# qirui-chen/RGA3-release

Measured on AMD Instinct MI355X. Metric: video-QA samples/sec (fwd+bwd) at 7B/16-frame — full RGA3 training step (Qwen2.5-VL-7B + SAM2-L + mask losses + AdamW), higher is better.
Workload: dtype bf16

## Files before the change

### include/rga3_hip.h

```cpp
#ifndef RGA3_HIP_H
#define RGA3_HIP_H

#include <stddef.h>
#include <stdint.h>

#ifdef __cplusplus
extern "C" {
#endif

#define RGA3_EINVAL (-22)

#define RGA3_BF16 0
#define RGA3_F32 1

#define RGA3_ACT_NONE 0
#define RGA3_ACT_GELU 1
#define RGA3_ACT_SWIGLU 2
#define RGA3_ACT_RELU 3

int rga3_version(void);
int rga3_last_error(char* buf, size_t n);

int rga3_gemm_bf16(const void* A, const void* W, const void* bias, const void* residual, const void* colscale, void* C, int64_t M, int64_t N,
                   int64_t K, int64_t lda, int64_t ldw, int64_t ldc, int64_t ldr, int act, int out_dtype, int tile,
                   void* workspace, int64_t workspace_bytes, void* stream);
int rga3_gemm_rms_bf16(const void* A, const void* W, const void* bias, const void* residual, void* C, int64_t M, int64_t N, int64_t K, int64_t lda,
                       int64_t ldw, int64_t ldc, int64_t ldr, int act, int tile, void* workspace, int64_t workspace_bytes, const uint64_t* row_sumsq_in,
                       int64_t norm_width, float eps, uint64_t* row_sumsq_out, void* stream);
int rga3_gemm_swiglu_pre_bf16(const void* A, const void* W, const void* bias, void* C, void* pre, int64_t M, int64_t N, int64_t K, int64_t lda, int64_t ldw,
                              int64_t ldc, int64_t ldpre, int tile, void* workspace, int64_t workspace_bytes, void* stream);
int rga3_gemm_cat_bf16(const void* A, const void* W, const void* bias, void* C, int64_t M, int64_t N, int64_t K, int64_t lda, int64_t ldw, int64_t ldc,
                       const void* A2, const void* W2, int64_t K2, int64_t lda2, int64_t ldw2, const void* Wn, void* Cn, int64_t N2, int64_t ldwn, int64_t ldcn,
                       int tile, void* stream);

int64_t rga3_gemm_workspace_bytes(void);
int rga3_gemm_tn_bf16(const void* A, const void* B, const void* bias, void* C, int64_t M, int64_t N, int64_t K, int64_t lda, int64_t ldb,
                      int64_t ldc, int out_dtype, void* workspace, int64_t workspace_bytes, void* counters, void* stream);
int rga3_gemm_tn_many(const void* const* ptrs, const int64_t* dims, int n, void* workspace, int64_t workspace_bytes, void* stream);


int rga3_attn_varlen_fwd(const void* q, const void* k, const void* v, void* o, float* lse, const int32_t* cu_q,
                         const int32_t* cu_k, int nseg, int max_q, int64_t total_q, int Hq, int Hkv, int D, int64_t q_st, int64_t q_sh,
                         int64_t k_st, int64_t k_sh, int64_t v_st, int64_t v_sh, int64_t o_st, int64_t o_sh,
                         float scale, int causal, int impl, float* split_ws, int64_t split_ws_elems, int max_k, int block_q, int block_k, void* stream);
int rga3_attn_varlen_fwd_rope(const void* q, const void* k, const void* v, void* o, float* lse, const int32_t* cu_q, const int32_t* cu_k, int nseg, int max_q,
                              int64_t total_q, int Hq, int Hkv, int D, int64_t q_st, int64_t q_sh, int64_t k_st, int64_t k_sh, int64_t v_st, int64_t v_sh,
                              int64_t o_st, int64_t o_sh, float scale, int causal, const float* cos_q, const float* sin_q, const float* cos_k,
                              const float* sin_k, void* stream);

int rga3_rmsnorm_fwd(const void* x, const void* add, const void* weight, void* y, void* res_out, int64_t rows,
                     int64_t dim, int64_t ldx, float eps, void* stream);

int rga3_layernorm_fwd(const void* x, const void* weight, const void* bias, void* y, int64_t rows, int64_t dim,
                       int64_t ldx, int64_t ldy, float eps, int act, void* stream);
int rga3_layernorm_stats(const void* x, float* stats, int64_t rows, int64_t dim, int64_t ldx, float eps, void* stream);
int rga3_gemm_ln_bf16(const void* A, const void* Wf, const void* bias, const float* colc, const float* rowstat, void* C, int64_t M, int64_t N, int64_t K,
                      int64_t lda, int64_t ldw, int64_t ldc, int act, int tile, void* stream);
int64_t rga3_gemm_lnsum_slices(int64_t N, int tile);
int rga3_gemm_lnsum_bf16(const void* A, const void* W, const void* bias, const void* residual, void* C, int64_t M, int64_t N, int64_t K, int64_t lda,
                         int64_t ldw, int64_t ldc, int64_t ldr, int tile, float* row_parts, void* stream);
int rga3_gemm_lnq_bf16(const void* A, const void* Wf, const void* bias, const float* colc, const float* row_parts, int64_t slices, int64_t norm_width, float eps,
                       void* C, int64_t M, int64_t N, int64_t K, int64_t lda, int64_t ldw, int64_t ldc, int act, int tile, void* stream);

int rga3_rope_inplace(void* x, const float* cos, const float* sin, int64_t T, int h0, int nh, int D, int64_t st,
                      int64_t sh, void* stream);

int rga3_gather_rows(const void* table, const int64_t* idx, void* out, int64_t n_idx, int64_t rows_per_idx,
                     int64_t dim, int64_t ld_table, int64_t ld_out, void* stream);
int rga3_scatter_rows(const void* src, const int64_t* idx, void* out, int64_t n_idx, int64_t rows_per_idx, int64_t dim,
                      int64_t ld_src, int64_t ld_out, void* stream);

int rga3_pad_cols(const void* src, void* dst, int64_t rows, int64_t cols, int64_t ld_src, int64_t ld_dst, void* stream);

int rga3_silu_mul(const void* a, const void* b, void* out, int64_t n, void* stream);
int rga3_add(const void* a, const void* b, void* out, int64_t n, void* stream);

int rga3_cross_entropy_rows(const void* logits, int logits_dtype, const int64_t* labels, float* row_loss,
                            void* dlogits, int64_t rows, int64_t V, int64_t ld, float grad_scale, void* stream);


int rga3_im2col(const void* img, void* out, int64_t F, int C, int H, int W, int ks, int stride, int pad, int64_t ld_out,
                void* stream);
int rga3_maxpool2x2_win(const void* x, void* y, int64_t nwin, int w, int C, int64_t ldx, int64_t ldy, void* stream);
int rga3_upsample2x_add(const void* a, const void* b, void* out, int64_t F, int H, int W, int C, void* stream);
int rga3_add_bcast(const void* a, const void* b, void* out, int64_t rows, int64_t rows_b, int C, int64_t lda, int64_t ldb,
                   int64_t ldo, float alpha, void* stream);
int rga3_bilinear(const void* in, int in_dtype, float* out, const int32_t* plane_idx, int64_t N, int Hi, int Wi, int Ho, int Wo,
                  void* stream);
int rga3_conv3x3s2(const void* x, int x_dtype, const void* w, const void* bias, void* y, int64_t F, int H, int W, int Cin, int Cout,
                   float sig_scale, float sig_bias, void* stream);
int rga3_decimg_rows(const void* keys, int64_t keys_stride, const void* pe, int64_t pe_stride, int hw, const void* kt, const void* vt, int nk, const void* wq, const void* bq,
                     const void* wo, const void* bo, const void* ln_w, const void* ln_b, float eps, const void* wk2, const void* bk2, const void* wv2, const void* bv2,
                     void* keys_out, int64_t keys_out_stride, void* k2, void* v2, int64_t kv_stride, int v2_transposed, float scale, int64_t M, void* stream);
int rga3_attn_fewq(const void* q, int64_t q_stride, const void* k, int64_t k_stride, int64_t k_head_stride, const void* vt, const void* vbias, void* out, int64_t out_stride,
                   int frames, int nq, int nk, int H, float scale, void* stream);
int rga3_copy_many(void* const* dst, const void* const* src, const int64_t* bytes, int n, void* stream);
int rga3_conv3x3s2_ln_gelu(const void* x, int x_dtype, const void* w, const void* bias, const void* ln_w, const void* ln_b, float eps, void* y, int64_t F, int H, int W,
                           int Cin, int Cout, float sig_scale, float sig_bias, void* stream);
int rga3_im2col3x3s2(const void* x, void* cols, int64_t F, int H, int W, int C, void* stream);
int rga3_dwconv7x7(const void* x, const void* w, const void* bias, void* y, int64_t F, int H, int W, int C, void* stream);
int rga3_rope_axial_inplace(void* x, const float* cos, const float* sin, int64_t n_rope, int nq, int C, int64_t ldx, void* stream);
int rga3_pixel_shuffle2x(const void* g, const void* bias, const void* add, void* out, int64_t F, int H, int W, int Co, int act, void* stream);
int rga3_bce_dice_sums(const float* logits, const float* targets, float* out4, int64_t n_masks, int64_t hw, void* stream);
int64_t rga3_bce_dice_sums_ws_floats(int64_t n_masks, int64_t hw);
int rga3_bce_dice_sums_det(const float* logits, const float* targets, float* out4, float* ws, int64_t ws_floats, int64_t n_masks, int64_t hw, void* stream);
int64_t rga3_mask_jf_ws_bytes(int64_t frames, int64_t h, int64_t w);
int rga3_mask_jf_counts(const void* seg, const void* ann, const void* void_pixels, int64_t* counts, void* ws, int64_t ws_bytes, int64_t frames, int64_t h, int64_t w,
                        int radius, void* stream);
int64_t rga3_stom_ws_bytes(int64_t frames, int64_t h, int64_t w);
int rga3_stom_flow(const float* tracks, const void* visibility, int* records, int64_t frames, int64_t n_points, int vip_frame_idx, void* stream);
int rga3_stom_shift_composite(const void* frames_u8, const void* overlay_rgba, const int* records, void* out, int64_t frames, int64_t h, int64_t w, int vip_frame_idx,
                              void* stream);
int rga3_stom_mask_composite(const void* frames_u8, const void* overlay_rgba, const float* tracks, const void* visibility, void* out, void* ws, int64_t ws_bytes,
                             int64_t frames, int64_t h, int64_t w, int64_t n_points, int vip_frame_idx, const void* spans, int ksize, const void* half_widths,
                             int radius, void* stream);


int rga3_attn_varlen_bwd(const void* q, const void* k, const void* v, const void* o, const void* dout, const float* lse, void* dq,
                         void* dk, void* dv, float* delta_ws, const int32_t* cu_q, const int32_t* cu_k, int nseg, int max_q,
                         int max_k, int64_t total_q, int Hq, int Hkv, int D, const int64_t* strides16, float scale, int causal,
                         float* dkv_ws, int64_t total_k, void* stream);
int rga3_hiera_mlp144(const void* x, const void* w1f, const float* c1, const void* d1, const void* w2, const void* b2, void* y, int64_t M, float eps, void* stream);
int64_t rga3_hiera_mlp288_pack_bytes(void);
int rga3_hiera_mlp288_pack(const void* w1f, const float* c1, const void* d1, const void* w2, void* pack, void* stream);
int rga3_hiera_mlp288(const void* x, const void* pack, const void* b2, void* y, int64_t M, float eps, void* stream);
int rga3_mlp3_rows(const void* const* ptrs, const int64_t* dims, int n, int64_t B, void* stream);
int rga3_sam_select_objptr(const void* iou, const void* obj, const void* toks, int64_t tok_bstride, int C, const void* w0, const void* b0, const void* w1, const void* b1,
                           const void* w2, const void* b2, const void* no_obj_ptr, int64_t* best, int32_t* sel, void* obj_ptr, int64_t B, void* stream);
int64_t rga3_memattn_cross_ws_floats(int64_t Nq, int nsplit);
int rga3_memattn_cross(const void* q, const void* k, const void* m, void* out, int64_t Nq, int64_t Nk, int64_t q_stride, int64_t k_stride, int64_t m_stride,
                       int64_t out_stride, float scale, int nsplit, float* ws, void* stream);
int rga3_memlayer_rows(const void* a, int64_t a_stride, int K1, const float* part_o, const float* part_ml, int nsplit, const void* w1, const void* b1,
                       const void* res, int64_t res_stride, void* x_out, int64_t x_stride, const void* ln_w, const void* ln_b, float eps, void* t_out,
                       int64_t t_stride, const void* w2, const void* b2, int N2, void* y_out, int64_t y_stride, const float* cos, const float* sin,
                       int rope_cols, int nq, int64_t M, void* stream);
int rga3_gemm_rows16_many(const void* const* ptrs, const int64_t* dims, int n, void* stream);
int rga3_gemm_stream_k_timeouts(const void* workspace);
int64_t rga3_gemm_timeout_counter_offset(void);
int rga3_gemm_ragged_plan(int64_t M, int64_t N, int64_t K, int cus, int split, int* plan, unsigned* start);
int rga3_gemm_tiles(int entry, int* ids, int* bm, int* bn, int cap);
int rga3_gemm_candidates(int entry, int64_t M, int64_t N, int64_t K, int act, int out_dtype, int epilogue, int* ids, int cap);
int rga3_gemm_tn_slices(int64_t M, int64_t N, int64_t K);
int rga3_rmsnorm_bwd(const void* x, const void* weight, const void* dy, const void* add, void* dx, int64_t rows, int64_t dim, float eps,
                     void* stream);
int rga3_dropout_bf16(const void* x, void* y, int64_t n, float p, int64_t seed, int accumulate, void* stream);
int rga3_dropout_pair_bf16(const void* xa, const void* xb, void* ya, void* yb, int64_t n, float pa, int64_t seed_a, float pb, int64_t seed_b, int sum, void* stream);
int rga3_swiglu_fwd(const void* gu, void* a, int64_t T, int64_t I, void* stream);
int rga3_swiglu_bwd(const void* gu, const void* da, void* dgu, int64_t T, int64_t I, void* stream);
int rga3_transpose16(const void* in, void* out, int64_t R, int64_t C, int64_t ld_in, int64_t ld_out, void* stream);
int rga3_transpose16_many(const void* const* ptrs, const int64_t* dims, int n, void* stream);
int rga3_segment_sum_rows(const void* x, const int64_t* rows, const int64_t* offsets, void* out, int64_t n_out, int64_t dim, int64_t ldx,
                          void* stream);
int rga3_adamw_step(void* param, float* master, const void* grad, float* m, float* v, int64_t n, float lr, float beta1, float beta2,
                    float eps, float weight_decay, int step, float grad_scale, void* stream);
int rga3_sumsq_accum(const void* g, float* out, int64_t n, void* stream);
int rga3_sumsq_det(const void* g, int64_t n, float* partials, int64_t partials_cap, float* out, int accumulate, void* stream);
int rga3_adamw_step_clip(void* param, float* master, const void* grad, float* m, float* v, int64_t n, float lr, float beta1, float beta2,
                         float eps, float weight_decay, int step, const float* sumsq, float max_norm, void* stream);
int rga3_adamw_step_clip_rows(void* param, float* master, const void* grad, float* m, float* v, int64_t rows, int64_t row_len, const uint8_t* row_active,
                              float lr, float beta1, float beta2, float eps, int step, const float* sumsq, float max_norm, void* stream);
int rga3_scatter_add_rows(void* dst, const int64_t* idx, const void* src, int64_t n, int64_t dim, int64_t ld_dst, int64_t ld_src, float scale,
                          void* stream);


int64_t rga3_layernorm_bwd_ws_floats(int64_t rows, int64_t dim);
int rga3_layernorm_bwd(const void* x, const void* weight, const void* dy, void* dx, float* dweight, float* dbias, int64_t rows, int64_t dim,
                       float eps, float* ws, int64_t ws_floats, void* stream);
int rga3_colsum_accum(const void* x, float* out, int64_t rows, int64_t cols, int64_t ld, void* stream);
int64_t rga3_colsum_ws_floats(int64_t rows, int64_t cols);
int rga3_colsum(const void* x, float* out, int64_t rows, int64_t cols, int64_t ld, float* ws, int64_t ws_floats, void* counters, void* stream);
int rga3_act(const void* a, const void* dy, void* out, int64_t n, int kind, void* stream);
int rga3_bilinear_bwd(const float* dout, float* din, const int32_t* plane_idx, int64_t N, int Hi, int Wi, int Ho, int Wo, void* stream);
int rga3_mask_product(const void* hyper, const void* up, float* masks, int64_t B, int64_t NM, int64_t P, int64_t C, void* stream);
int64_t rga3_mask_product_bwd_ws_floats(int64_t B, int64_t NM, int64_t P, int64_t C);
int rga3_mask_product_bwd(const float* dmasks, const void* hyper, const void* up, void* dup, void* dhyper, int64_t B, int64_t NM, int64_t P, int64_t C,
                          float* ws, int64_t ws_floats, void* stream);
int rga3_pixel_shuffle2x_bwd(const void* dout, void* dg, int64_t F, int H, int W, int Co, void* stream);
int rga3_bce_dice_grad(const float* logits, const float* targets, const float* sums4, float* dlogits, int64_t n_masks, int64_t hw,
                       float coef_bce, float coef_dice, void* stream);
int rga3_bce_dice_grad_dev(const float* logits, const float* targets, const float* sums4, float* dlogits, int64_t n_masks, int64_t hw,
                           const float* coef_bce_dev, const float* coef_dice_dev, void* stream);

int rga3_pil_bicubic_coeffs(int in_size, int out_size, int32_t* bounds, int32_t* kk, int64_t kk_capacity, int* ksize_out);
int rga3_sam_preprocess_u8(const void* frames, int64_t T, int H, int W, int out_h, int out_w, const int32_t* bh, const int32_t* kh,
                           int ksize_h, const int32_t* bv, const int32_t* kv, int ksize_v, void* tmp, void* dst_u8, void* dst_bf16,
                           const float* mean3, const float* std3, void* stream);

int rga3_qwen_norm_lut(const float* mean3, const float* std3, int fused, float* lut768);
int rga3_qwen_patchify_u8(const void* frames, int64_t T, int h, int w, const float* lut768, void* out, int out_dtype, int patch, int tpatch,
                          int merge, void* stream);

int rga3_quant_fp8_rows(const void* x, void* q, float* scales, int64_t rows, int64_t K, int64_t ldx, int64_t ldq, void* stream);
int rga3_gemm_fp8(const void* Aq, const void* Wq, const float* sa, const float* sw, const void* bias, const void* residual, void* C, int64_t M,
                  int64_t N, int64_t K, int64_t lda, int64_t ldw, int64_t ldc, int64_t ldr, void* stream);
int rga3_swiglu_fwd_quant_fp8(const void* gu, void* q, float* scales, int64_t T, int64_t I, void* stream);
int rga3_swiglu_bwd_quant_fp8(const void* gu, const void* da, void* q, float* scales, int64_t T, int64_t I, void* stream);

#ifdef __cplusplus
}
#endif
#endif
```

### rga3-release_amd/csrc/attn_bwd.hip

```cpp
#include "common.h"

namespace rga3 {

struct AttnBwdArgs {
    const unsigned short *q, *k, *v, *o, *dout;
    unsigned short *dq, *dk, *dv;
    const float* lse;
    float* delta;
    const int *cu_q, *cu_k;
    long q_st, q_sh, k_st, k_sh, v_st, v_sh, o_st, o_sh, do_st, do_sh, dq_st, dq_sh, dk_st, dk_sh, dv_st, dv_sh;
    int Hq, Hkv, D;
    long total_q;
    float scale, scale_log2;
    int causal;
    float* dkv_ws;
    long total_k;
    int gx, gy;
};

constexpr int BT = 64;

template <int DP, int QT, int NWAVE, bool PAIR>
__global__ __launch_bounds__(64 * NWAVE) void attn_bwd_dq_kernel(AttnBwdArgs p) {
    constexpr int NT = 64 * NWAVE;
    constexpr int BLOCK_M = NWAVE * QT * 16;
    constexpr int CH = DP / 8;
    constexpr int STRIDE = DP * 2 + 32;
    constexpr int DS = DP / 32, DT = DP / 16;
    constexpr int LOADS = (BT * CH) / NT;
    static_assert((BT * CH) % NT == 0, "tile chunks must divide evenly over threads");

    extern __shared__ __attribute__((aligned(16))) char smem[];
    char* Ks = smem;
    char* Vs = smem + BT * STRIDE;

    const int tid = threadIdx.x, lane = tid & 63;
    const int wid = __builtin_amdgcn_readfirstlane(tid >> 6);
    const int g = lane >> 4, c = lane & 15;
    const Wg3 wg = xcd_decode3(p.gx, p.gy);
    const int seg = wg.z, hq = wg.y;
    const int hk = hq / (p.Hq / p.Hkv);
    const int qs = p.cu_q[seg], Lq = p.cu_q[seg + 1] - qs;
    const int ks = p.cu_k[seg], Lk = p.cu_k[seg + 1] - ks;
    const int shift = Lk - Lq;
    const int nqb = (Lq + BLOCK_M - 1) / BLOCK_M;
    int qb_first = wg.x, qb_second = -1;
    if constexpr (PAIR) {
        qb_first = nqb - 1 - wg.x;
        qb_second = wg.x;
        if (qb_second > qb_first) return;
        if (qb_second == qb_first) qb_second = -1;
    } else if (qb_first >= nqb) {
        return;
    }
    for (int pass = 0; pass < (PAIR ? 2 : 1); ++pass) {
    const int qbi = pass == 0 ? qb_first : qb_second;
    if (qbi < 0) break;
    if (pass == 1) __syncthreads();
    const int qb0 = qbi * BLOCK_M;
    const int qw0 = qb0 + wid * (QT * 16);

    bf16x8 qf[QT][DS], dof[QT][DS];
    float lse2[QT], dl[QT];
#pragma unroll
    for (int t = 0; t < QT; ++t) {
        const int qi = qw0 + t * 16 + c;
        const bool ok = qi < Lq;
#pragma unroll
        for (int ds = 0; ds < DS; ++ds) {
            const int d = ds * 32 + g * 8;
            u32x4 z = {0u, 0u, 0u, 0u}, y = {0u, 0u, 0u, 0u};
            if (ok && d < p.D) {
                z = *(const u32x4*)(p.q + (long)(qs + qi) * p.q_st + (long)hq * p.q_sh + d);
                y = *(const u32x4*)(p.dout + (long)(qs + qi) * p.do_st + (long)hq * p.do_sh + d);
            }
            qf[t][ds] = __builtin_bit_cast(bf16x8, z);
            dof[t][ds] = __builtin_bit_cast(bf16x8, y);
        }
        lse2[t] = ok ? p.lse[(long)hq * p.total_q + qs + qi] * 1.4426950408889634f : 0.f;
    }
#pragma unroll
    for (int t = 0; t < QT; ++t) {
        const int qi = qw0 + t * 16 + c;
        const bool ok = qi < Lq;
        float dp = 0.f;
#pragma unroll
        for (int ds = 0; ds < DS; ++ds) {
            const int d = ds * 32 + g * 8;
            if (ok && d < p.D) {
                const u32x4 ov = *(const u32x4*)(p.o + (long)(qs + qi) * p.o_st + (long)hq * p.o_sh + d);
                const u32x4 dv = __builtin_bit_cast(u32x4, dof[t][ds]);
#pragma unroll
                for (int i = 0; i < 4; ++i) {
                    dp += __uint_as_float(ov[i] << 16) * __uint_as_float(dv[i] << 16);
                    dp += __uint_as_float(ov[i] & 0xffff0000u) * __uint_as_float(dv[i] & 0xffff0000u);
                }
            }
        }
        dp += __shfl_xor(dp, 16, 64);
        dp += __shfl_xor(dp, 32, 64);
        dl[t] = ok ? dp : 0.f;
        if (ok && g == 0) p.delta[(long)hq * p.total_q + qs + qi] = dp;
    }

    f32x4 dqacc[QT][DT];
#pragma unroll
    for (int t = 0; t < QT; ++t)
#pragma unroll
        for (int d = 0; d < DT; ++d) dqacc[t][d] = f32x4{0.f, 0.f, 0.f, 0.f};

    int kv_end = Lk;
    if (p.causal) kv_end = min(Lk, qb0 + BLOCK_M + shift);
    if (kv_end < 0) kv_end = 0;
    const int ntiles = (kv_end + BT - 1) / BT;

    u32x4 kreg[LOADS], vreg[LOADS];
    auto load_tile = [&](int kt) {
#pragma unroll
        for (int i = 0; i < LOADS; ++i) {
            const int idx = tid + i * NT;
            const int r = idx / CH, ch = idx % CH;
            const int key = kt * BT + r;
            u32x4 zk = {0u, 0u, 0u, 0u}, zv = {0u, 0u, 0u, 0u};
            if (key < Lk && ch * 8 < p.D) {
                zk = *(const u32x4*)(p.k + (long)(ks + key) * p.k_st + (long)hk * p.k_sh + ch * 8);
                zv = *(const u32x4*)(p.v + (long)(ks + key) * p.v_st + (long)hk * p.v_sh + ch * 8);
            }
            kreg[i] = zk;
            vreg[i] = zv;
        }
    };
    auto store_tile = [&]() {
#pragma unroll
        for (int i = 0; i < LOADS; ++i) {
            const int idx = tid + i * NT;
            const int r = idx / CH, ch = idx % CH;
            *(u32x4*)(Ks + r * STRIDE + ch * 16) = kreg[i];
            *(u32x4*)(Vs + r * STRIDE + ch * 16) = vreg[i];
        }
    };

    if (ntiles > 0) load_tile(0);
    for (int kt = 0; kt < ntiles; ++kt) {
        __syncthreads();
        store_tile();
        __syncthreads();
        if (kt + 1 < ntiles) load_tile(kt + 1);
        const int k0 = kt * BT;
        const bool need_mask = (k0 + BT > Lk) || (p.causal && (k0 + BT - 1 > qb0 + shift));
#pragma unroll
        for (int t = 0; t < QT; ++t) {
            const int qi = qw0 + t * 16 + c;
            f32x4 s[4], dp[4];
#pragma unroll
            for (int j = 0; j < 4; ++j) { s[j] = f32x4{0.f, 0.f, 0.f, 0.f}; dp[j] = f32x4{0.f, 0.f, 0.f, 0.f}; }
#pragma unroll
            for (int j = 0; j < 4; ++j)
#pragma unroll
                for (int ds = 0; ds < DS; ++ds) {
                    bf16x8 kf = *(const bf16x8*)(Ks + (j * 16 + c) * STRIDE + ds * 64 + g * 16);
                    bf16x8 vf = *(const bf16x8*)(Vs + (j * 16 + c) * STRIDE + ds * 64 + g * 16);
                    s[j] = __builtin_amdgcn_mfma_f32_16x16x32_bf16(kf, qf[t][ds], s[j], 0, 0, 0);
                    dp[j] = __builtin_amdgcn_mfma_f32_16x16x32_bf16(vf, dof[t][ds], dp[j], 0, 0, 0);
                }
            bf16x8 dsf[2];
#pragma unroll
            for (int ss = 0; ss < 2; ++ss) {
                float e[8];
#pragma unroll
                for (int u = 0; u < 8; ++u) {
                    const int j = 2 * ss + (u >> 2), r = u & 3;
                    float pr = __builtin_amdgcn_exp2f(s[j][r] * p.scale_log2 - lse2[t]);
                    if (need_mask) {
                        const int key = k0 + j * 16 + 4 * g + r;
                        const bool ok = (key < Lk) && (!p.causal || key <= qi + shift);
                        pr = ok ? pr : 0.f;
                    }
                    if (qi >= Lq) pr = 0.f;
                    e[u] = pr * (dp[j][r] - dl[t]) * p.scale;
                }
                u32x4 pk;
                pk[0] = pack_bf2(e[0], e[1]); pk[1] = pack_bf2(e[2], e[3]); pk[2] = pack_bf2(e[4], e[5]); pk[3] = pack_bf2(e[6], e[7]);
                dsf[ss] = __builtin_bit_cast(bf16x8, pk);
            }
#pragma unroll
            for (int d = 0; d < DT; ++d)
#pragma unroll
                for (int ss = 0; ss < 2; ++ss) {
                    const char* a0 = Ks + (ss * 32 + 4 * g + (c >> 2)) * STRIDE + (d * 16 + 4 * (c & 3)) * 2;
                    bf16x4 lo = __builtin_amdgcn_ds_read_tr16_b64_v4bf16((__attribute__((address_space(3))) bf16x4*)(a0));
                    bf16x4 hi = __builtin_amdgcn_ds_read_tr16_b64_v4bf16((__attribute__((address_space(3))) bf16x4*)(a0 + 16 * STRIDE));
                    bf16x8 kt8;
                    kt8[0] = lo[0]; kt8[1] = lo[1]; kt8[2] = lo[2]; kt8[3] = lo[3];
                    kt8[4] = hi[0]; kt8[5] = hi[1]; kt8[6] = hi[2]; kt8[7] = hi[3];
                    dqacc[t][d] = __builtin_amdgcn_mfma_f32_16x16x32_bf16(kt8, dsf[ss], dqacc[t][d], 0, 0, 0);
                }
        }
    }
#pragma unroll
    for (int t = 0; t < QT; ++t) {
        const int qi = qw0 + t * 16 + c;
        if (qi < Lq) {
            unsigned short* row = p.dq + (long)(qs + qi) * p.dq_st + (long)hq * p.dq_sh;
#pragma unroll
            for (int d = 0; d < DT; ++d) {
                const int dd = d * 16 + 4 * g;
                if (dd < p.D) {
                    u32x2 pk;
                    pk[0] = pack_bf2(dqacc[t][d][0], dqacc[t][d][1]);
                    pk[1] = pack_bf2(dqacc[t][d][2], dqacc[t][d][3]);
                    *(u32x2*)(row + dd) = pk;
                }
            }
        }
    }
    }
}

template <int DP, int NWAVE, bool SPLIT, bool PAIR>
__global__ __launch_bounds__(64 * NWAVE) void attn_bwd_dkv_kernel(AttnBwdArgs p) {
    constexpr int NT = 64 * NWAVE;
    constexpr int BLOCK_N = NWAVE * 16;
    constexpr int CH = DP / 8;
    constexpr int STRIDE = DP * 2 + 32;
    constexpr int DS = DP / 32, DT = DP / 16;
    constexpr int LOADS = (BT * CH) / NT;
    static_assert((BT * CH) % NT == 0, "tile chunks must divide evenly over threads");

    extern __shared__ __attribute__((aligned(16))) char smem[];
    char* Qs = smem;
    char* Os = smem + BT * STRIDE;
    float* Ls = (float*)(smem + 2 * BT * STRIDE);

    const int tid = threadIdx.x, lane = tid & 63;
    const int wid = __builtin_amdgcn_readfirstlane(tid >> 6);
    const int g = lane >> 4, c = lane & 15;
    const Wg3 wg = xcd_decode3(p.gx, p.gy);
    const int seg = wg.z;
    const int group = p.Hq / p.Hkv;
    const int hk = SPLIT ? wg.y / group : wg.y;
    const int hh0 = SPLIT ? wg.y % group : 0, hh1 = SPLIT ? hh0 + 1 : group;
    const int qs = p.cu_q[seg], Lq = p.cu_q[seg + 1] - qs;
    const int ks = p.cu_k[seg], Lk = p.cu_k[seg + 1] - ks;
    const int shift = Lk - Lq;
    const int nkb = (Lk + BLOCK_N - 1) / BLOCK_N;
    int kb_first = wg.x, kb_second = -1;
    if constexpr (PAIR) {
        kb_first = wg.x;
        kb_second = nkb - 1 - wg.x;
        if (kb_first > kb_second) return;
        if (kb_second == kb_first) kb_second = -1;
    } else if (kb_first >= nkb) {
        return;
    }
    for (int pass = 0; pass < (PAIR ? 2 : 1); ++pass) {
    const int kbi = pass == 0 ? kb_first : kb_second;
    if (kbi < 0) break;
    if (pass == 1) __syncthreads();
    const int kb0 = kbi * BLOCK_N;
    const int key = kb0 + wid * 16 + c;

    bf16x8 kf[DS], vf[DS];
#pragma unroll
    for (int ds = 0; ds < DS; ++ds) {
        const int d = ds * 32 + g * 8;
        u32x4 z = {0u, 0u, 0u, 0u}, y = {0u, 0u, 0u, 0u};
        if (key < Lk && d < p.D) {
            z = *(const u32x4*)(p.k + (long)(ks + key) * p.k_st + (long)hk * p.k_sh + d);
            y = *(const u32x4*)(p.v + (long)(ks + key) * p.v_st + (long)hk * p.v_sh + d);
        }
        kf[ds] = __builtin_bit_cast(bf16x8, z);
        vf[ds] = __builtin_bit_cast(bf16x8, y);
    }
    f32x4 dkacc[DT], dvacc[DT];
#pragma unroll
    for (int d = 0; d < DT; ++d) { dkacc[d] = f32x4{0.f, 0.f, 0.f, 0.f}; dvacc[d] = f32x4{0.f, 0.f, 0.f, 0.f}; }

    int q_begin = 0;
    if (p.causal) q_begin = max(0, kb0 - shift);
    const int t0 = q_begin / BT;
    const int ntq = (Lq + BT - 1) / BT;

    u32x4 qreg[LOADS], oreg[LOADS];
    float lreg = 0.f, dreg = 0.f;
    auto load_tile = [&](int hq_, int qt_) {
#pragma unroll
        for (int i = 0; i < LOADS; ++i) {
            const int idx = tid + i * NT;
            const int r = idx / CH, ch = idx % CH;
            const int qi = qt_ * BT + r;
            u32x4 zq = {0u, 0u, 0u, 0u}, zo = {0u, 0u, 0u, 0u};
            if (qi < Lq && ch * 8 < p.D) {
                zq = *(const u32x4*)(p.q + (long)(qs + qi) * p.q_st + (long)hq_ * p.q_sh + ch * 8);
                zo = *(const u32x4*)(p.dout + (long)(qs + qi) * p.do_st + (long)hq_ * p.do_sh + ch * 8);
            }
            qreg[i] = zq;
            oreg[i] = zo;
        }
        if (tid < BT) {
            const int qi = qt_ * BT + tid;
            lreg = (qi < Lq) ? p.lse[(long)hq_ * p.total_q + qs + qi] * 1.4426950408889634f : 0.f;
            dreg = (qi < Lq) ? p.delta[(long)hq_ * p.total_q + qs + qi] : 0.f;
        }
    };
    auto store_tile = [&]() {
#pragma unroll
        for (int i = 0; i < LOADS; ++i) {
            const int idx = tid + i * NT;
            const int r = idx / CH, ch = idx % CH;
            *(u32x4*)(Qs + r * STRIDE + ch * 16) = qreg[i];
            *(u32x4*)(Os + r * STRIDE + ch * 16) = oreg[i];
        }
        if (tid < BT) {
            Ls[tid] = lreg;
            Ls[BT + tid] = dreg;
        }
    };
    if (t0 < ntq) load_tile(hk * group + hh0, t0);
    for (int hh = hh0; hh < hh1; ++hh) {
        const int hq = hk * group + hh;
        for (int qt = t0; qt < ntq; ++qt) {
            __syncthreads();
            store_tile();
            __syncthreads();
            if (qt + 1 < ntq) load_tile(hq, qt + 1);
            else if (hh + 1 < hh1) load_tile(hq + 1, t0);
            const int q0 = qt * BT;
            f32x4 s[4], dp[4];
#pragma unroll
            for (int j = 0; j < 4; ++j) { s[j] = f32x4{0.f, 0.f, 0.f, 0.f}; dp[j] = f32x4{0.f, 0.f, 0.f, 0.f}; }
#pragma unroll
            for (int j = 0; j < 4; ++j)
#pragma unroll
                for (int ds = 0; ds < DS; ++ds) {
                    bf16x8 qa = *(const bf16x8*)(Qs + (j * 16 + c) * STRIDE + ds * 64 + g * 16);
                    bf16x8 oa = *(const bf16x8*)(Os + (j * 16 + c) * STRIDE + ds * 64 + g * 16);
                    s[j] = __builtin_amdgcn_mfma_f32_16x16x32_bf16(qa, kf[ds], s[j], 0, 0, 0);
                    dp[j] = __builtin_amdgcn_mfma_f32_16x16x32_bf16(oa, vf[ds], dp[j], 0, 0, 0);
                }
            bf16x8 pf[2], dsf[2];
#pragma unroll
            for (int ss = 0; ss < 2; ++ss) {
                float e[8], f[8];
#pragma unroll
                for (int u = 0; u < 8; ++u) {
                    const int j = 2 * ss + (u >> 2), r = u & 3;
                    const int ql = j * 16 + 4 * g + r;
                    const int qi = q0 + ql;
                    float pr = __builtin_amdgcn_exp2f(s[j][r] * p.scale_log2 - Ls[ql]);
                    const bool ok = (qi < Lq) && (key < Lk) && (!p.causal || key <= qi + shift);
                    pr = ok ? pr : 0.f;
                    e[u] = pr;
                    f[u] = pr * (dp[j][r] - Ls[BT + ql]) * p.scale;
                }
                u32x4 a, b;
                a[0] = pack_bf2(e[0], e[1]); a[1] = pack_bf2(e[2], e[3]); a[2] = pack_bf2(e[4], e[5]); a[3] = pack_bf2(e[6], e[7]);
                b[0] = pack_bf2(f[0], f[1]); b[1] = pack_bf2(f[2], f[3]); b[2] = pack_bf2(f[4], f[5]); b[3] = pack_bf2(f[6], f[7]);
                pf[ss] = __builtin_bit_cast(bf16x8, a);
                dsf[ss] = __builtin_bit_cast(bf16x8, b);
            }
#pragma unroll
            for (int d = 0; d < DT; ++d)
#pragma unroll
                for (int ss = 0; ss < 2; ++ss) {
                    const int roff = (ss * 32 + 4 * g + (c >> 2)) * STRIDE + (d * 16 + 4 * (c & 3)) * 2;
                    bf16x4 ol = __builtin_amdgcn_ds_read_tr16_b64_v4bf16((__attribute__((address_space(3))) bf16x4*)(Os + roff));
                    bf16x4 oh = __builtin_amdgcn_ds_read_tr16_b64_v4bf16((__attribute__((address_space(3))) bf16x4*)(Os + roff + 16 * STRIDE));
                    bf16x4 ql_ = __builtin_amdgcn_ds_read_tr16_b64_v4bf16((__attribute__((address_space(3))) bf16x4*)(Qs + roff));
                    bf16x4 qh_ = __builtin_amdgcn_ds_read_tr16_b64_v4bf16((__attribute__((address_space(3))) bf16x4*)(Qs + roff + 16 * STRIDE));
                    bf16x8 ot, qt8;
                    ot[0] = ol[0]; ot[1] = ol[1]; ot[2] = ol[2]; ot[3] = ol[3]; ot[4] = oh[0]; ot[5] = oh[1]; ot[6] = oh[2]; ot[7] = oh[3];
                    qt8[0] = ql_[0]; qt8[1] = ql_[1]; qt8[2] = ql_[2]; qt8[3] = ql_[3]; qt8[4] = qh_[0]; qt8[5] = qh_[1]; qt8[6] = qh_[2]; qt8[7] = qh_[3];
                    dvacc[d] = __builtin_amdgcn_mfma_f32_16x16x32_bf16(ot, pf[ss], dvacc[d], 0, 0, 0);
                    dkacc[d] = __builtin_amdgcn_mfma_f32_16x16x32_bf16(qt8, dsf[ss], dkacc[d], 0, 0, 0);
                }
        }
    }
    if constexpr (SPLIT) {
        if (key < Lk) {
            const long half = (long)group * p.total_k * p.Hkv * p.D;
            float* wk = p.dkv_ws + (((long)hh0 * p.total_k + ks + key) * p.Hkv + hk) * p.D;
#pragma unroll
            for (int d = 0; d < DT; ++d) {
                const int dd = d * 16 + 4 * g;
                if (dd < p.D) {
                    *(f32x4*)(wk + dd) = dkacc[d];
                    *(f32x4*)(wk + half + dd) = dvacc[d];
                }
            }
        }
        continue;
    }
    if (key < Lk) {
        unsigned short* rk = p.dk + (long)(ks + key) * p.dk_st + (long)hk * p.dk_sh;
        unsigned short* rv = p.dv + (long)(ks + key) * p.dv_st + (long)hk * p.dv_sh;
#pragma unroll
        for (int d = 0; d < DT; ++d) {
            const int dd = d * 16 + 4 * g;
            if (dd < p.D) {
                u32x2 a, b;
                a[0] = pack_bf2(dkacc[d][0], dkacc[d][1]); a[1] = pack_bf2(dkacc[d][2], dkacc[d][3]);
                b[0] = pack_bf2(dvacc[d][0], dvacc[d][1]); b[1] = pack_bf2(dvacc[d][2], dvacc[d][3]);
                *(u32x2*)(rk + dd) = a;
                *(u32x2*)(rv + dd) = b;
            }
        }
    }
    }
}

__global__ __launch_bounds__(256) void attn_dkv_reduce_kernel(AttnBwdArgs p) {
    const int group = p.Hq / p.Hkv;
    const int d4 = p.D / 4;
    const long idx = (long)blockIdx.x * 256 + threadIdx.x;
    const long total = p.total_k * p.Hkv * d4;
    if (idx >= total) return;
    const int dd = (int)(idx % d4) * 4;
    const long row = idx / d4;
    const int hk = (int)(row % p.Hkv);
    const long key = row / p.Hkv;
    const long plane = p.total_k * p.Hkv * (long)p.D, half = (long)group * plane;
    const float* w = p.dkv_ws + row * p.D + dd;
    f32x4 sk = *(const f32x4*)w, sv = *(const f32x4*)(w + half);
    for (int h = 1; h < group; ++h) {
        sk += *(const f32x4*)(w + h * plane);
        sv += *(const f32x4*)(w + half + h * plane);
    }
    u32x2 a, b;
    a[0] = pack_bf2(sk[0], sk[1]); a[1] = pack_bf2(sk[2], sk[3]);
    b[0] = pack_bf2(sv[0], sv[1]); b[1] = pack_bf2(sv[2], sv[3]);
    *(u32x2*)(p.dk + key * p.dk_st + (long)hk * p.dk_sh + dd) = a;
    *(u32x2*)(p.dv + key * p.dv_st + (long)hk * p.dv_sh + dd) = b;
}

template <auto K>
static int launch_bwd_grid(AttnBwdArgs& a, int lds, unsigned gx, int gy, int nseg, int nwave, hipStream_t st, const char* name) {
    a.gx = (int)gx; a.gy = gy;
    return launch_lds<K>(dim3(gx * (unsigned)gy * (unsigned)nseg), dim3(64 * nwave), lds, st, name, a);
}

template <int DP>
static int launch_bwd(const AttnBwdArgs& a0, int nseg, int max_q, int max_k, hipStream_t st) {
    AttnBwdArgs a = a0;
    a.gx = 1; a.gy = 1;
    constexpr int NW = (DP == 128) ? 8 : 4;
#ifdef RGA3_BWD_DQ_QT2
    constexpr int QT = 2, NWQ = 4;
#else
    constexpr int QT = (DP >= 128) ? 1 : 2, NWQ = NW;
#endif
    constexpr int BLOCK_M = NWQ * QT * 16;
    constexpr int LDS_DQ = 2 * BT * (DP * 2 + 32);
    constexpr int LDS_DKV = 2 * BT * (DP * 2 + 32) + 2 * BT * 4;
    const unsigned nqb = (unsigned)cdiv(max_q, BLOCK_M), nkb = (unsigned)cdiv(max_k, 16 * NW);
    const bool pair = a.causal && nqb >= 4 && nkb >= 4;
    const unsigned gq = pair ? (nqb + 1) / 2 : nqb, gk = pair ? (nkb + 1) / 2 : nkb;
    if (int rc = pair ? launch_bwd_grid<attn_bwd_dq_kernel<DP, QT, NWQ, true>>(a, LDS_DQ, gq, a.Hq, nseg, NWQ, st, "attn_bwd_dq_kernel")
                      : launch_bwd_grid<attn_bwd_dq_kernel<DP, QT, NWQ, false>>(a, LDS_DQ, gq, a.Hq, nseg, NWQ, st, "attn_bwd_dq_kernel"))
        return rc;
    if (a.dkv_ws && a.Hq > a.Hkv) {
        if (int rc = pair ? launch_bwd_grid<attn_bwd_dkv_kernel<DP, NW, true, true>>(a, LDS_DKV, gk, a.Hq, nseg, NW, st, "attn_bwd_dkv_kernel<split>")
                          : launch_bwd_grid<attn_bwd_dkv_kernel<DP, NW, true, false>>(a, LDS_DKV, gk, a.Hq, nseg, NW, st, "attn_bwd_dkv_kernel<split>"))
            return rc;
        const long rows = a.total_k * a.Hkv;
        hipLaunchKernelGGL(attn_dkv_reduce_kernel, dim3((unsigned)cdiv(rows * (a.D / 4), 256)), dim3(256), 0, st, a);
        RGA3_CHECK_LAUNCH("attn_dkv_reduce_kernel");
        return 0;
    }
    return pair ? launch_bwd_grid<attn_bwd_dkv_kernel<DP, NW, false, true>>(a, LDS_DKV, gk, a.Hkv, nseg, NW, st, "attn_bwd_dkv_kernel")
                : launch_bwd_grid<attn_bwd_dkv_kernel<DP, NW, false, false>>(a, LDS_DKV, gk, a.Hkv, nseg, NW, st, "attn_bwd_dkv_kernel");
}

}

using namespace rga3;

extern "C" int rga3_attn_varlen_bwd(const void* q, const void* k, const void* v, const void* o, const void* dout, const float* lse,
                                    void* dq, void* dk, void* dv, float* delta_ws, const int32_t* cu_q, const int32_t* cu_k, int nseg,
                                    int max_q, int max_k, int64_t total_q, int Hq, int Hkv, int D, const int64_t* strides16, float scale,
                                    int causal, float* dkv_ws, int64_t total_k, void* stream) {
    RGA3_CHECK_ARG(q && k && v && o && dout && lse && dq && dk && dv && delta_ws && cu_q && cu_k && strides16, "attn_bwd: null pointer");
    RGA3_CHECK_ARG(nseg > 0 && max_q > 0 && max_k > 0 && total_q > 0, "attn_bwd: sizes");
    RGA3_CHECK_ARG(Hq > 0 && Hkv > 0 && Hq % Hkv == 0, "attn_bwd: Hq=%d Hkv=%d", Hq, Hkv);
    RGA3_CHECK_ARG(D >= 8 && D <= 128 && D % 8 == 0, "attn_bwd: head dim %d unsupported (multiple of 8, <= 128)", D);
    for (int i = 0; i < 16; ++i) RGA3_CHECK_ARG(strides16[i] % 4 == 0, "attn_bwd: stride %d must be a multiple of 4 elements", i);
    for (int i = 0; i < 10; ++i) RGA3_CHECK_ARG(strides16[i] % 8 == 0, "attn_bwd: input stride %d must be a multiple of 8 elements", i);
    {
        static const char* const names[8] = {"q", "k", "v", "o", "dout", "dq", "dk", "dv"};
        for (int i = 0; i < 8; ++i) {
            const bool kv = i == 1 || i == 2 || i == 6 || i == 7;
            RGA3_CHECK_HEADS("attn_bwd", names[i], strides16[2 * i], strides16[2 * i + 1], kv ? total_k : total_q, kv ? Hkv : Hq, D);
        }
    }
    AttnBwdArgs a;
    a.q = (const unsigned short*)q; a.k = (const unsigned short*)k; a.v = (const unsigned short*)v; a.o = (const unsigned short*)o;
    a.dout = (const unsigned short*)dout; a.dq = (unsigned short*)dq; a.dk = (unsigned short*)dk; a.dv = (unsigned short*)dv;
    a.lse = lse; a.delta = delta_ws; a.cu_q = cu_q; a.cu_k = cu_k;
    a.q_st = strides16[0]; a.q_sh = strides16[1]; a.k_st = strides16[2]; a.k_sh = strides16[3]; a.v_st = strides16[4]; a.v_sh = strides16[5];
    a.o_st = strides16[6]; a.o_sh = strides16[7]; a.do_st = strides16[8]; a.do_sh = strides16[9]; a.dq_st = strides16[10]; a.dq_sh = strides16[11];
    a.dk_st = strides16[12]; a.dk_sh = strides16[13]; a.dv_st = strides16[14]; a.dv_sh = strides16[15];
    a.Hq = Hq; a.Hkv = Hkv; a.D = D; a.total_q = total_q; a.scale = scale; a.scale_log2 = scale * 1.4426950408889634f; a.causal = causal;
    a.dkv_ws = dkv_ws; a.total_k = total_k;
    RGA3_CHECK_ARG(!dkv_ws || (total_k > 0 && D % 4 == 0), "attn_bwd: dkv_ws needs total_k");
    hipStream_t st = (hipStream_t)stream;
    if (D <= 32) return launch_bwd<32>(a, nseg, max_q, max_k, st);
    if (D <= 64) return launch_bwd<64>(a, nseg, max_q, max_k, st);
    if (D <= 96) return launch_bwd<96>(a, nseg, max_q, max_k, st);
    return launch_bwd<128>(a, nseg, max_q, max_k, st);
}
```

### rga3-release_amd/csrc/trainops.hip

```cpp
#include "common.h"

namespace rga3 {

template <int MAXC>
__global__ __launch_bounds__(256) void rmsnorm_bwd_kernel(const unsigned short* __restrict__ x, const unsigned short* __restrict__ w,
                                                          const unsigned short* __restrict__ dy, const unsigned short* __restrict__ add,
                                                          unsigned short* __restrict__ dx, long rows, int dim, float eps) {
    const int lane = threadIdx.x & 63;
    const long row = (long)blockIdx.x * 4 + (threadIdx.x >> 6);
    if (row >= rows) return;
    const int nch = dim / 8;
    u32x4 xb[MAXC], gb[MAXC];
    float ss = 0.f, sg = 0.f;
#pragma unroll
    for (int i = 0; i < MAXC; ++i) {
        const int ch = lane + i * 64;
        if (ch < nch) {
            float fx[8], fd[8], fw[8];
            xb[i] = *(const u32x4*)(x + row * dim + ch * 8);
            unpack8(xb[i], fx);
            unpack8(*(const u32x4*)(dy + row * dim + ch * 8), fd);
            unpack8(*(const u32x4*)(w + ch * 8), fw);
#pragma unroll
            for (int e = 0; e < 8; ++e) {
                fd[e] *= fw[e];
                ss += fx[e] * fx[e];
                sg += fd[e] * fx[e];
            }
            gb[i] = pack8(fd);
        }
    }
    ss = wave_sum(ss);
    sg = wave_sum(sg);
    const float r = rsqrtf(ss / (float)dim + eps);
    const float coef = r * r * r * sg / (float)dim;
#pragma unroll
    for (int i = 0; i < MAXC; ++i) {
        const int ch = lane + i * 64;
        if (ch < nch) {
            float fx[8], fg[8], fa[8];
            unpack8(xb[i], fx);
            unpack8(gb[i], fg);
            if (add) unpack8(*(const u32x4*)(add + row * dim + ch * 8), fa);
#pragma unroll
            for (int e = 0; e < 8; ++e) fg[e] = r * fg[e] - fx[e] * coef + (add ? fa[e] : 0.f);
            *(u32x4*)(dx + row * dim + ch * 8) = pack8(fg);
        }
    }
}

template <int NC>
__global__ __launch_bounds__(256) void rmsnorm_bwd_block_kernel(const unsigned short* __restrict__ x, const unsigned short* __restrict__ w,
                                                                const unsigned short* __restrict__ dy, const unsigned short* __restrict__ add,
                                                                unsigned short* __restrict__ dx, int dim, float eps) {
    __shared__ float red[2][4];
    const int lane = threadIdx.x & 63, wv = threadIdx.x >> 6;
    const long row = blockIdx.x;
    const int nch = dim / 8;
    float fx[NC][8], fg[NC][8];
    float ss = 0.f, sg = 0.f;
#pragma unroll
    for (int i = 0; i < NC; ++i) {
        const int ch = threadIdx.x + i * 256;
        if (ch < nch) {
            float fw[8];
            unpack8(*(const u32x4*)(x + row * dim + ch * 8), fx[i]);
            unpack8(*(const u32x4*)(dy + row * dim + ch * 8), fg[i]);
            unpack8(*(const u32x4*)(w + ch * 8), fw);
#pragma unroll
            for (int e = 0; e < 8; ++e) {
                fg[i][e] *= fw[e];
                ss += fx[i][e] * fx[i][e];
                sg += fg[i][e] * fx[i][e];
            }
        }
    }
    ss = wave_sum(ss);
    sg = wave_sum(sg);
    if (lane == 0) { red[0][wv] = ss; red[1][wv] = sg; }
    __syncthreads();
    ss = (red[0][0] + red[0][1]) + (red[0][2] + red[0][3]);
    sg = (red[1][0] + red[1][1]) + (red[1][2] + red[1][3]);
    const float r = rsqrtf(ss / (float)dim + eps);
    const float coef = r * r * r * sg / (float)dim;
#pragma unroll
    for (int i = 0; i < NC; ++i) {
        const int ch = threadIdx.x + i * 256;
        if (ch < nch) {
            float fa[8], o[8];
            if (add) unpack8(*(const u32x4*)(add + row * dim + ch * 8), fa);
#pragma unroll
            for (int e = 0; e < 8; ++e) o[e] = r * fg[i][e] - fx[i][e] * coef + (add ? fa[e] : 0.f);
            *(u32x4*)(dx + row * dim + ch * 8) = pack8(o);
        }
    }
}

__global__ __launch_bounds__(256) void swiglu_bwd_kernel(const unsigned short* __restrict__ gu, const unsigned short* __restrict__ da,
                                                         unsigned short* __restrict__ dgu, long T, long I) {
    const long nch = I / 8;
    const long total = T * nch;
    for (long i = (long)blockIdx.x * 256 + threadIdx.x; i < total; i += (long)gridDim.x * 256) {
        const long ch = i % nch, t = i / nch;
        const long blk = ch / 2, half = ch % 2;
        const long goff = t * 2 * I + blk * 32 + half * 8;
        float g[8], u[8], d[8], dg[8], du[8];
        unpack8(*(const u32x4*)(gu + goff), g);
        unpack8(*(const u32x4*)(gu + goff + 16), u);
        unpack8(*(const u32x4*)(da + t * I + ch * 8), d);
#pragma unroll
        for (int e = 0; e < 8; ++e) swiglu_bwd_elem(g[e], u[e], d[e], dg[e], du[e]);
        *(u32x4*)(dgu + goff) = pack8(dg);
        *(u32x4*)(dgu + goff + 16) = pack8(du);
    }
}

__global__ __launch_bounds__(256) void swiglu_fwd_kernel(const unsigned short* __restrict__ gu, unsigned short* __restrict__ a, long T, long I) {
    const long nch = I / 8;
    const long total = T * nch;
    for (long i = (long)blockIdx.x * 256 + threadIdx.x; i < total; i += (long)gridDim.x * 256) {
        const long ch = i % nch, t = i / nch;
        const long blk = ch / 2, half = ch % 2;
        const long goff = t * 2 * I + blk * 32 + half * 8;
        float g[8], u[8], o[8];
        unpack8(*(const u32x4*)(gu + goff), g);
        unpack8(*(const u32x4*)(gu + goff + 16), u);
#pragma unroll
        for (int e = 0; e < 8; ++e) o[e] = swiglu_fwd_elem(g[e], u[e]);
        *(u32x4*)(a + t * I + ch * 8) = pack8(o);
    }
}

__global__ __launch_bounds__(256) void transpose16_kernel(const unsigned short* __restrict__ in, unsigned short* __restrict__ out, long R, long C,
                                                          long ldi, long ldo) {
    __shared__ unsigned short tile[64][66];
    const long r0 = (long)blockIdx.y * 64, c0 = (long)blockIdx.x * 64;
    const int tx = threadIdx.x & 63, ty = threadIdx.x >> 6;
    for (int i = ty; i < 64; i += 4) {
        const long r = r0 + i, c = c0 + tx;
        tile[i][tx] = (r < R && c < C) ? in[r * ldi + c] : (unsigned short)0;
    }
    __syncthreads();
    for (int i = ty; i < 64; i += 4) {
        const long c = c0 + i, r = r0 + tx;
        if (c < C && r < R) out[c * ldo + r] = tile[tx][i];
    }
}

constexpr int TR_MANY = 64;
struct TransposeMany {
    const unsigned short* in[TR_MANY];
    unsigned short* out[TR_MANY];
    int R[TR_MANY], C[TR_MANY];
};
__global__ __launch_bounds__(256) void transpose16_many_kernel(TransposeMany p) {
    __shared__ unsigned short tile[64][66];
    const int m = blockIdx.z;
    const long R = p.R[m], C = p.C[m];
    const long r0 = (long)blockIdx.y * 64, c0 = (long)blockIdx.x * 64;
    if (r0 >= R || c0 >= C) return;
    const unsigned short* in = p.in[m];
    unsigned short* out = p.out[m];
    const int tx = threadIdx.x & 63, ty = threadIdx.x >> 6;
    for (int i = ty; i < 64; i += 4) {
        const long r = r0 + i, c = c0 + tx;
        tile[i][tx] = (r < R && c < C) ? in[r * C + c] : (unsigned short)0;
    }
    __syncthreads();
    for (int i = ty; i < 64; i += 4) {
        const long c = c0 + i, r = r0 + tx;
        if (c < C && r < R) out[c * R + r] = tile[tx][i];
    }
}

__global__ __launch_bounds__(256) void segment_sum_rows_kernel(const unsigned short* __restrict__ x, const long* __restrict__ rows,
                                                               const long* __restrict__ off, unsigned short* __restrict__ out, int dim, long ldx) {
    const long u = blockIdx.x;
    const long a = off[u], b = off[u + 1];
    for (int ch = threadIdx.x; ch < dim / 8; ch += 256) {
        float acc[8] = {0, 0, 0, 0, 0, 0, 0, 0};
        for (long j = a; j < b; ++j) {
            float f[8];
            unpack8(*(const u32x4*)(x + rows[j] * ldx + ch * 8), f);
#pragma unroll
            for (int e = 0; e < 8; ++e) acc[e] += f[e];
        }
        *(u32x4*)(out + u * dim + ch * 8) = pack8(acc);
    }
}

__global__ __launch_bounds__(256) void adamw_kernel(unsigned short* __restrict__ p, float* __restrict__ master, const unsigned short* __restrict__ g,
                                                    float* __restrict__ m, float* __restrict__ v, long n, float lr, float b1, float b2, float eps,
                                                    float wd, float bc1, float bc2, float gscale) {
    for (long i = (long)blockIdx.x * 256 + threadIdx.x; i < n; i += (long)gridDim.x * 256) {
        const float gr = bf2f(g[i]) * gscale;
        float w = master[i];
        const float mi = b1 * m[i] + (1.f - b1) * gr;
        const float vi = b2 * v[i] + (1.f - b2) * gr * gr;
        m[i] = mi;
        v[i] = vi;
        w = w * (1.f - lr * wd) - lr * (mi / bc1) / (sqrtf(vi / bc2) + eps);
        master[i] = w;
        p[i] = f2bf(w);
    }
}

__global__ __launch_bounds__(256) void sumsq_kernel(const unsigned short* __restrict__ g, float* __restrict__ out, long n) {
    __shared__ float red[4];
    float s = 0.f;
    for (long i = (long)blockIdx.x * 256 + threadIdx.x; i < n; i += (long)gridDim.x * 256) {
        const float x = bf2f(g[i]);
        s += x * x;
    }
    s = wave_sum(s);
    if ((threadIdx.x & 63) == 0) red[threadIdx.x >> 6] = s;
    __syncthreads();
    if (threadIdx.x == 0) atomicAdd(out, red[0] + red[1] + red[2] + red[3]);
}

__global__ __launch_bounds__(256) void sumsq_partials_kernel(const unsigned short* __restrict__ g, float* __restrict__ partials, long n) {
    __shared__ float red[4];
    float s = 0.f;
    const long n8 = n / 8;
    for (long i = (long)blockIdx.x * 256 + threadIdx.x; i < n8; i += (long)gridDim.x * 256) {
        float f[8];
        unpack8(*(const u32x4*)(g + i * 8), f);
#pragma unroll
        for (int e = 0; e < 8; ++e) s += f[e] * f[e];
    }
    if (blockIdx.x == 0 && threadIdx.x < (n & 7)) {
        const float x = bf2f(g[n8 * 8 + threadIdx.x]);
        s += x * x;
    }
    s = wave_sum(s);
    if ((threadIdx.x & 63) == 0) red[threadIdx.x >> 6] = s;
    __syncthreads();
    if (threadIdx.x == 0) partials[blockIdx.x] = (red[0] + red[1]) + (red[2] + red[3]);
}

__global__ __launch_bounds__(256) void sumsq_finish_kernel(const float* __restrict__ partials, int np, float* __restrict__ out, int accumulate) {
    __shared__ float red[256];
    float s = 0.f;
    for (int i = threadIdx.x; i < np; i += 256) s += partials[i];
    red[threadIdx.x] = s;
    __syncthreads();
    for (int o = 128; o > 0; o >>= 1) {
        if ((int)threadIdx.x < o) red[threadIdx.x] += red[threadIdx.x + o];
        __syncthreads();
    }
    if (threadIdx.x == 0) out[0] = (accumulate ? out[0] : 0.f) + red[0];
}

__global__ __launch_bounds__(256) void adamw8_kernel(unsigned short* __restrict__ p, float* __restrict__ master, const unsigned short* __restrict__ g,
                                                     float* __restrict__ m, float* __restrict__ v, long n, float lr, float b1, float b2, float eps,
                                                     float wd, float bc1, float bc2, const float* __restrict__ sumsq, float max_norm,
                                                     const unsigned char* __restrict__ row_active, long row_len8) {
    float gscale = 1.f;
    if (sumsq) gscale = fminf(1.f, max_norm / (sqrtf(sumsq[0]) + 1e-6f));
    const long n8 = n / 8;
    const float decay = 1.f - lr * wd, ibc1 = 1.f / bc1, ibc2 = 1.f / bc2;
    for (long i = (long)blockIdx.x * 256 + threadIdx.x; i < n8; i += (long)gridDim.x * 256) {
        if (row_active && !row_active[i / row_len8]) continue;
        float gr[8], w[8], mi[8], vi[8];
        unpack8(*(const u32x4*)(g + i * 8), gr);
        *(f32x4*)(w) = *(const f32x4*)(master + i * 8);     *(f32x4*)(w + 4) = *(const f32x4*)(master + i * 8 + 4);
        *(f32x4*)(mi) = *(const f32x4*)(m + i * 8);         *(f32x4*)(mi + 4) = *(const f32x4*)(m + i * 8 + 4);
        *(f32x4*)(vi) = *(const f32x4*)(v + i * 8);         *(f32x4*)(vi + 4) = *(const f32x4*)(v + i * 8 + 4);
#pragma unroll
        for (int e = 0; e < 8; ++e) {
            const float x = gr[e] * gscale;
            mi[e] = b1 * mi[e] + (1.f - b1) * x;
            vi[e] = b2 * vi[e] + (1.f - b2) * x * x;
            w[e] = w[e] * decay - lr * (mi[e] * ibc1) / (sqrtf(vi[e] * ibc2) + eps);
        }
        *(f32x4*)(master + i * 8) = *(f32x4*)(w);           *(f32x4*)(master + i * 8 + 4) = *(f32x4*)(w + 4);
        *(f32x4*)(m + i * 8) = *(f32x4*)(mi);               *(f32x4*)(m + i * 8 + 4) = *(f32x4*)(mi + 4);
        *(f32x4*)(v + i * 8) = *(f32x4*)(vi);               *(f32x4*)(v + i * 8 + 4) = *(f32x4*)(vi + 4);
        *(u32x4*)(p + i * 8) = pack8(w);
    }
    if (blockIdx.x == 0 && threadIdx.x < (n & 7)) {
        const long i = n8 * 8 + threadIdx.x;
        const float x = bf2f(g[i]) * gscale;
        const float mm = b1 * m[i] + (1.f - b1) * x, vv = b2 * v[i] + (1.f - b2) * x * x;
        const float w = master[i] * decay - lr * (mm * ibc1) / (sqrtf(vv * ibc2) + eps);
        m[i] = mm; v[i] = vv; master[i] = w; p[i] = f2bf(w);
    }
}

__global__ __launch_bounds__(256) void scatter_add_rows_kernel(unsigned short* __restrict__ dst, const long* __restrict__ idx, const unsigned short* __restrict__ src,
                                                               long n, int dim, long ld_dst, long ld_src, float scale) {
    const int nch = dim / 8;
    for (long t = (long)blockIdx.x * 256 + threadIdx.x; t < n * nch; t += (long)gridDim.x * 256) {
        const long r = t / nch;
        const int ch = (int)(t % nch);
        float a[8], b[8];
        unsigned short* d = dst + idx[r] * ld_dst + ch * 8;
        unpack8(*(const u32x4*)d, a);
        unpack8(*(const u32x4*)(src + r * ld_src + ch * 8), b);
#pragma unroll
        for (int e = 0; e < 8; ++e) a[e] += scale * b[e];
        *(u32x4*)d = pack8(a);
    }
}

__device__ __forceinline__ unsigned dropout_hash(unsigned long long seed, unsigned long long ctr) {
    unsigned x = (unsigned)ctr ^ (unsigned)seed, y = (unsigned)(ctr >> 32) ^ (unsigned)(seed >> 32);
    x *= 0xcc9e2d51u; x = (x << 15) | (x >> 17); x *= 0x1b873593u;
    y ^= x; y = (y << 13) | (y >> 19); y = y * 5u + 0xe6546b64u;
    y ^= y >> 16; y *= 0x85ebca6bu; y ^= y >> 13; y *= 0xc2b2ae35u; y ^= y >> 16;
    return y;
}

__global__ __launch_bounds__(256) void dropout_kernel(const unsigned short* __restrict__ x, unsigned short* __restrict__ y, long n8, unsigned thr,
                                                      float inv_keep, unsigned long long seed, int accumulate) {
    for (long g = (long)blockIdx.x * 256 + threadIdx.x; g < n8; g += (long)gridDim.x * 256) {
        const u32x4 v = *(const u32x4*)(x + g * 8);
        u32x4 o = {0u, 0u, 0u, 0u};
        if (accumulate) o = *(const u32x4*)(y + g * 8);
#pragma unroll
        for (int j = 0; j < 4; ++j) {
            const unsigned h = dropout_hash(seed, (unsigned long long)g * 4 + j);
            const float lo = ((h & 0xffffu) >= thr) ? __uint_as_float(v[j] << 16) * inv_keep : 0.f;
            const float hi = ((h >> 16) >= thr) ? __uint_as_float(v[j] & 0xffff0000u) * inv_keep : 0.f;
            const float alo = accumulate ? __uint_as_float(o[j] << 16) : 0.f, ahi = accumulate ? __uint_as_float(o[j] & 0xffff0000u) : 0.f;
            o[j] = pack_bf2(alo + lo, ahi + hi);
        }
        *(u32x4*)(y + g * 8) = o;
    }
}

__global__ __launch_bounds__(256) void dropout_pair_kernel(const unsigned short* __restrict__ xa, const unsigned short* __restrict__ xb, unsigned short* ya,
                                                           unsigned short* yb, long n8, unsigned thr_a, float ik_a, unsigned long long seed_a, unsigned thr_b,
                                                           float ik_b, unsigned long long seed_b, int sum) {
    const bool same = xa == xb;
    for (long g = (long)blockIdx.x * 256 + threadIdx.x; g < n8; g += (long)gridDim.x * 256) {
        const u32x4 va = *(const u32x4*)(xa + g * 8);
        const u32x4 vb = same ? va : *(const u32x4*)(xb + g * 8);
        u32x4 o = {0u, 0u, 0u, 0u};
        if (sum) o = *(const u32x4*)(ya + g * 8);
        u32x4 oa, ob;
#pragma unroll
        for (int j = 0; j < 4; ++j) {
            const unsigned ha = dropout_hash(seed_a, (unsigned long long)g * 4 + j), hb = dropout_hash(seed_b, (unsigned long long)g * 4 + j);
            const float alo = ((ha & 0xffffu) >= thr_a) ? __uint_as_float(va[j] << 16) * ik_a : 0.f;
            const float ahi = ((ha >> 16) >= thr_a) ? __uint_as_float(va[j] & 0xffff0000u) * ik_a : 0.f;
            const float blo = ((hb & 0xffffu) >= thr_b) ? __uint_as_float(vb[j] << 16) * ik_b : 0.f;
            const float bhi = ((hb >> 16) >= thr_b) ? __uint_as_float(vb[j] & 0xffff0000u) * ik_b : 0.f;
            if (sum) {
                oa[j] = pack_bf2(__uint_as_float(o[j] << 16) + alo + blo, __uint_as_float(o[j] & 0xffff0000u) + ahi + bhi);
            } else {
                oa[j] = pack_bf2(alo, ahi);
                ob[j] = pack_bf2(blo, bhi);
            }
        }
        *(u32x4*)(ya + g * 8) = oa;
        if (!sum) *(u32x4*)(yb + g * 8) = ob;
    }
}

}

using namespace rga3;

extern "C" int rga3_rmsnorm_bwd(const void* x, const void* weight, const void* dy, const void* add, void* dx, int64_t rows, int64_t dim,
                                float eps, void* stream) {
    RGA3_CHECK_ARG(x && weight && dy && dx && rows > 0 && dim > 0 && dim % 8 == 0 && dim <= 8192, "rmsnorm_bwd: bad args");
    hipStream_t st = (hipStream_t)stream;
    if (dim > 1024) {
        dim3 gb((unsigned)rows);
        if (dim <= 2048) hipLaunchKernelGGL(rmsnorm_bwd_block_kernel<1>, gb, dim3(256), 0, st, (cus)x, (cus)weight, (cus)dy, (cus)add, (us)dx, (int)dim, eps);
        else if (dim <= 4096) hipLaunchKernelGGL(rmsnorm_bwd_block_kernel<2>, gb, dim3(256), 0, st, (cus)x, (cus)weight, (cus)dy, (cus)add, (us)dx, (int)dim, eps);
        else hipLaunchKernelGGL(rmsnorm_bwd_block_kernel<4>, gb, dim3(256), 0, st, (cus)x, (cus)weight, (cus)dy, (cus)add, (us)dx, (int)dim, eps);
        RGA3_CHECK_LAUNCH("rmsnorm_bwd_block");
        return 0;
    }
    dim3 grid((unsigned)cdiv(rows, 4));
    if (dim <= 2048) hipLaunchKernelGGL(rmsnorm_bwd_kernel<4>, grid, dim3(256), 0, st, (cus)x, (cus)weight, (cus)dy, (cus)add, (us)dx, (long)rows, (int)dim, eps);
    else if (dim <= 4096) hipLaunchKernelGGL(rmsnorm_bwd_kernel<8>, grid, dim3(256), 0, st, (cus)x, (cus)weight, (cus)dy, (cus)add, (us)dx, (long)rows, (int)dim, eps);
    else hipLaunchKernelGGL(rmsnorm_bwd_kernel<16>, grid, dim3(256), 0, st, (cus)x, (cus)weight, (cus)dy, (cus)add, (us)dx, (long)rows, (int)dim, eps);
    RGA3_CHECK_LAUNCH("rmsnorm_bwd");
    return 0;
}

extern "C" int rga3_dropout_bf16(const void* x, void* y, int64_t n, float p, int64_t seed, int accumulate, void* stream) {
    RGA3_CHECK_ARG(x && y && n > 0 && n % 8 == 0, "dropout: n=%ld must be a positive multiple of 8", (long)n);
    RGA3_CHECK_ARG(p >= 0.f && p < 1.f, "dropout: p=%f", p);
    const unsigned thr = (unsigned)(p * 65536.0f + 0.5f);
    const float inv_keep = 1.0f / (1.0f - (float)thr / 65536.0f);
    long blocks = cdiv(n / 8, 256);
    if (blocks > 65536) blocks = 65536;
    hipLaunchKernelGGL(dropout_kernel, dim3((unsigned)blocks), dim3(256), 0, (hipStream_t)stream, (const unsigned short*)x, (unsigned short*)y, (long)(n / 8),
                       thr, inv_keep, (unsigned long long)seed, accumulate);
    RGA3_CHECK_LAUNCH("dropout_kernel");
    return 0;
}

extern "C" int rga3_dropout_pair_bf16(const void* xa, const void* xb, void* ya, void* yb, int64_t n, float pa, int64_t seed_a, float pb, int64_t seed_b, int sum,
                                      void* stream) {
    RGA3_CHECK_ARG(xa && xb && ya && (sum || yb) && n > 0 && n % 8 == 0, "dropout_pair: null pointer / n=%ld must be a positive multiple of 8", (long)n);
    RGA3_CHECK_ARG(pa >= 0.f && pa < 1.f && pb >= 0.f && pb < 1.f, "dropout_pair: p=%f / %f", pa, pb);
    RGA3_CHECK_ARG((((uintptr_t)xa | (uintptr_t)xb | (uintptr_t)ya | (uintptr_t)yb) & 15) == 0, "dropout_pair: pointers must be 16-byte aligned");
    const unsigned ta = (unsigned)(pa * 65536.0f + 0.5f), tb = (unsigned)(pb * 65536.0f + 0.5f);
    long blocks = cdiv(n / 8, 256);
    if (blocks > 65536) blocks = 65536;
    hipLaunchKernelGGL(dropout_pair_kernel, dim3((unsigned)blocks), dim3(256), 0, (hipStream_t)stream, (cus)xa, (cus)xb, (us)ya, (us)yb, (long)(n / 8), ta,
                       1.0f / (1.0f - (float)ta / 65536.0f), (unsigned long long)seed_a, tb, 1.0f / (1.0f - (float)tb / 65536.0f), (unsigned long long)seed_b, sum);
    RGA3_CHECK_LAUNCH("dropout_pair_kernel");
    return 0;
}

extern "C" int rga3_swiglu_bwd(const void* gu, const void* da, void* dgu, int64_t T, int64_t I, void* stream) {
    RGA3_CHECK_ARG(gu && da && dgu && T > 0 && I > 0 && I % 16 == 0, "swiglu_bwd: bad args");
    hipLaunchKernelGGL(swiglu_bwd_kernel, dim3(grid1d(T * (I / 8))), dim3(256), 0, (hipStream_t)stream, (cus)gu, (cus)da, (us)dgu, (long)T, (long)I);
    RGA3_CHECK_LAUNCH("swiglu_bwd");
    return 0;
}

extern "C" int rga3_swiglu_fwd(const void* gu, void* a, int64_t T, int64_t I, void* stream) {
    RGA3_CHECK_ARG(gu && a && T > 0 && I > 0 && I % 16 == 0, "swiglu_fwd: bad args");
    hipLaunchKernelGGL(swiglu_fwd_kernel, dim3(grid1d(T * (I / 8))), dim3(256), 0, (hipStream_t)stream, (cus)gu, (us)a, (long)T, (long)I);
    RGA3_CHECK_LAUNCH("swiglu_fwd");
    return 0;
}

extern "C" int rga3_transpose16(const void* in, void* out, int64_t R, int64_t C, int64_t ld_in, int64_t ld_out, void* stream) {
    RGA3_CHECK_ARG(in && out && R > 0 && C > 0, "transpose16: bad args");
    RGA3_CHECK_LD("transpose16", "ld_in", ld_in, C, 2);
    RGA3_CHECK_LD("transpose16", "ld_out", ld_out, R, 2);
    RGA3_CHECK_ARG(cdiv(R, 64) <= 65535, "transpose16: too many rows");
    hipLaunchKernelGGL(transpose16_kernel, dim3((unsigned)cdiv(C, 64), (unsigned)cdiv(R, 64)), dim3(256), 0, (hipStream_t)stream, (cus)in, (us)out, (long)R,
                       (long)C, (long)ld_in, (long)ld_out);
    RGA3_CHECK_LAUNCH("transpose16");
    return 0;
}

extern "C" int rga3_transpose16_many(const void* const* ptrs, const int64_t* dims, int n, void* stream) {
    RGA3_CHECK_ARG(ptrs && dims && n >= 1 && n <= TR_MANY, "transpose16_many: n %d (1..64)", n);
    TransposeMany p;
    long mr = 0, mc = 0;
    for (int i = 0; i < n; ++i) {
        p.in[i] = (const unsigned short*)ptrs[2 * i];
        p.out[i] = (unsigned short*)ptrs[2 * i + 1];
        RGA3_CHECK_ARG(p.in[i] && p.out[i] && dims[2 * i] > 0 && dims[2 * i + 1] > 0 && dims[2 * i] < (1 << 30) && dims[2 * i + 1] < (1 << 30), "transpose16_many: matrix %d", i);
        p.R[i] = (int)dims[2 * i];
        p.C[i] = (int)dims[2 * i + 1];
        if (p.R[i] > mr) mr = p.R[i];
        if (p.C[i] > mc) mc = p.C[i];
    }
    RGA3_CHECK_ARG(cdiv(mr, 64) <= 65535, "transpose16_many: too many rows");
    hipLaunchKernelGGL(transpose16_many_kernel, dim3((unsigned)cdiv(mc, 64), (unsigned)cdiv(mr, 64), (unsigned)n), dim3(256), 0, (hipStream_t)stream, p);
    RGA3_CHECK_LAUNCH("transpose16_many");
    return 0;
}

extern "C" int rga3_segment_sum_rows(const void* x, const int64_t* rows, const int64_t* offsets, void* out, int64_t n_out, int64_t dim,
                                     int64_t ldx, void* stream) {
    RGA3_CHECK_ARG(x && rows && offsets && out && n_out > 0 && dim % 8 == 0 && ldx % 8 == 0, "segment_sum_rows: bad args");
    RGA3_CHECK_LD("segment_sum_rows", "ldx", ldx, dim, 2);
    hipLaunchKernelGGL(segment_sum_rows_kernel, dim3((unsigned)n_out), dim3(256), 0, (hipStream_t)stream, (cus)x, (const long*)rows, (const long*)offsets,
                       (us)out, (int)dim, (long)ldx);
    RGA3_CHECK_LAUNCH("segment_sum_rows");
    return 0;
}

extern "C" int rga3_adamw_step(void* param, float* master, const void* grad, float* m, float* v, int64_t n, float lr, float beta1, float beta2,
                               float eps, float weight_decay, int step, float grad_scale, void* stream) {
    RGA3_CHECK_ARG(param && master && grad && m && v && n > 0 && step >= 1, "adamw_step: bad args");
    const float bc1 = 1.f - powf(beta1, (float)step), bc2 = 1.f - powf(beta2, (float)step);
    hipLaunchKernelGGL(adamw_kernel, dim3(grid1d(n)), dim3(256), 0, (hipStream_t)stream, (us)param, master, (cus)grad, m, v, (long)n, lr, beta1, beta2, eps,
                       weight_decay, bc1, bc2, grad_scale);
    RGA3_CHECK_LAUNCH("adamw_step");
    return 0;
}

extern "C" int rga3_sumsq_accum(const void* g, float* out, int64_t n, void* stream) {
    RGA3_CHECK_ARG(g && out && n > 0, "sumsq_accum: bad args");
    hipLaunchKernelGGL(sumsq_kernel, dim3(grid1d(n, 256, 2048)), dim3(256), 0, (hipStream_t)stream, (cus)g, out, (long)n);
    RGA3_CHECK_LAUNCH("sumsq_accum");
    return 0;
}

extern "C" int rga3_sumsq_det(const void* g, int64_t n, float* partials, int64_t partials_cap, float* out, int accumulate, void* stream) {
    RGA3_CHECK_ARG(g && partials && out && n > 0 && partials_cap >= 1, "sumsq_det: bad args");
    RGA3_CHECK_ARG(((uintptr_t)g & 15) == 0, "sumsq_det: gradient pointer must be 16-byte aligned");
    long nb = cdiv(n, 8 * 256 * 4);
    if (nb < 1) nb = 1;
    if (nb > partials_cap) nb = partials_cap;
    if (nb > 2048) nb = 2048;
    hipLaunchKernelGGL(sumsq_partials_kernel, dim3((unsigned)nb), dim3(256), 0, (hipStream_t)stream, (cus)g, partials, (long)n);
    RGA3_CHECK_LAUNCH("sumsq_partials");
    hipLaunchKernelGGL(sumsq_finish_kernel, dim3(1), dim3(256), 0, (hipStream_t)stream, (const float*)partials, (int)nb, out, accumulate);
    RGA3_CHECK_LAUNCH("sumsq_finish");
    return 0;
}

extern "C" int rga3_adamw_step_clip(void* param, float* master, const void* grad, float* m, float* v, int64_t n, float lr, float beta1, float beta2,
                                    float eps, float weight_decay, int step, const float* sumsq, float max_norm, void* stream) {
    RGA3_CHECK_ARG(param && master && grad && m && v && n > 0 && step >= 1, "adamw_step_clip: bad args");
    RGA3_CHECK_ARG((((uintptr_t)param | (uintptr_t)grad | (uintptr_t)master | (uintptr_t)m | (uintptr_t)v) & 15) == 0, "adamw_step_clip: pointers must be 16-byte aligned");
    const float bc1 = 1.f - powf(beta1, (float)step), bc2 = 1.f - powf(beta2, (float)step);
    hipLaunchKernelGGL(adamw8_kernel, dim3(grid1d(cdiv(n, 8), 256, 256L * 16)), dim3(256), 0, (hipStream_t)stream, (us)param, master, (cus)grad, m, v, (long)n, lr, beta1, beta2,
                       eps, weight_decay, bc1, bc2, sumsq, max_norm, (const unsigned char*)nullptr, 1L);
    RGA3_CHECK_LAUNCH("adamw_step_clip");
    return 0;
}

extern "C" int rga3_adamw_step_clip_rows(void* param, float* master, const void* grad, float* m, float* v, int64_t rows, int64_t row_len, const uint8_t* row_active,
                                         float lr, float beta1, float beta2, float eps, int step, const float* sumsq, float max_norm, void* stream) {
    RGA3_CHECK_ARG(param && master && grad && m && v && row_active && rows > 0 && row_len > 0 && row_len % 8 == 0 && step >= 1, "adamw_step_clip_rows: bad args (row_len % 8)");
    RGA3_CHECK_ARG((((uintptr_t)param | (uintptr_t)grad | (uintptr_t)master | (uintptr_t)m | (uintptr_t)v) & 15) == 0, "adamw_step_clip_rows: pointers must be 16-byte aligned");
    const float bc1 = 1.f - powf(beta1, (float)step), bc2 = 1.f - powf(beta2, (float)step);
    const int64_t n = rows * row_len;
    hipLaunchKernelGGL(adamw8_kernel, dim3(grid1d(cdiv(n, 8), 256, 256L * 16)), dim3(256), 0, (hipStream_t)stream, (us)param, master, (cus)grad, m, v, (long)n, lr, beta1, beta2,
                       eps, 0.f, bc1, bc2, sumsq, max_norm, row_active, (long)(row_len / 8));
    RGA3_CHECK_LAUNCH("adamw_step_clip_rows");
    return 0;
}

extern "C" int rga3_scatter_add_rows(void* dst, const int64_t* idx, const void* src, int64_t n, int64_t dim, int64_t ld_dst, int64_t ld_src, float scale,
                                     void* stream) {
    RGA3_CHECK_ARG(dst && idx && src && n > 0 && dim > 0 && dim % 8 == 0 && ld_dst % 8 == 0 && ld_src % 8 == 0, "scatter_add_rows: bad args");
    RGA3_CHECK_LD("scatter_add_rows", "ld_dst", ld_dst, dim, 2);
    RGA3_CHECK_LD("scatter_add_rows", "ld_src", ld_src, dim, n);
    hipLaunchKernelGGL(scatter_add_rows_kernel, dim3(grid1d(n * (dim / 8))), dim3(256), 0, (hipStream_t)stream, (us)dst, (const long*)idx, (cus)src, (long)n, (int)dim,
                       (long)ld_dst, (long)ld_src, scale);
    RGA3_CHECK_LAUNCH("scatter_add_rows");
    return 0;
}
```

### rga3-release_amd/rga3/hip/lib.py

```python
from __future__ import annotations

import ctypes as C
import os

_HERE = os.path.dirname(os.path.abspath(__file__))
LIB_PATH = os.path.normpath(os.path.join(_HERE, "..", "..", "librga3_hip.so"))

_p, _i, _i64, _f, _sz = C.c_void_p, C.c_int, C.c_int64, C.c_float, C.c_size_t

SIGNATURES = {
    "rga3_version": [],
    "rga3_last_error": [C.c_char_p, _sz],
    "rga3_gemm_bf16": [_p, _p, _p, _p, _p, _p, _i64, _i64, _i64, _i64, _i64, _i64, _i64, _i, _i, _i, _p, _i64, _p],
    "rga3_gemm_rms_bf16": [_p, _p, _p, _p, _p, _i64, _i64, _i64, _i64, _i64, _i64, _i64, _i, _i, _p, _i64, _p, _i64, _f, _p, _p],
    "rga3_gemm_workspace_bytes": [],
    "rga3_gemm_tn_bf16": [_p, _p, _p, _p, _i64, _i64, _i64, _i64, _i64, _i64, _i, _p, _i64, _p, _p],
    "rga3_gemm_tn_many": [_p, _p, _i, _p, _i64, _p],
    "rga3_gemm_swiglu_pre_bf16": [_p, _p, _p, _p, _p, _i64, _i64, _i64, _i64, _i64, _i64, _i64, _i, _p, _i64, _p],
    "rga3_gemm_cat_bf16": [_p, _p, _p, _p, _i64, _i64, _i64, _i64, _i64, _i64, _p, _p, _i64, _i64, _i64, _p, _p, _i64, _i64, _i64, _i, _p],
    "rga3_attn_varlen_fwd": [_p, _p, _p, _p, _p, _p, _p, _i, _i, _i64, _i, _i, _i, _i64, _i64, _i64, _i64, _i64, _i64,
                             _i64, _i64, _f, _i, _i, _p, _i64, _i, _i, _i, _p],
    "rga3_attn_varlen_fwd_rope": [_p, _p, _p, _p, _p, _p, _p, _i, _i, _i64, _i, _i, _i, _i64, _i64, _i64, _i64, _i64, _i64, _i64, _i64, _f, _i, _p, _p, _p, _p, _p],
    "rga3_rmsnorm_fwd": [_p, _p, _p, _p, _p, _i64, _i64, _i64, _f, _p],
    "rga3_layernorm_fwd": [_p, _p, _p, _p, _i64, _i64, _i64, _i64, _f, _i, _p],
    "rga3_layernorm_stats": [_p, _p, _i64, _i64, _i64, _f, _p],
    "rga3_gemm_ln_bf16": [_p, _p, _p, _p, _p, _p, _i64, _i64, _i64, _i64, _i64, _i64, _i, _i, _p],
    "rga3_gemm_lnsum_slices": [_i64, _i],
    "rga3_gemm_lnsum_bf16": [_p, _p, _p, _p, _p, _i64, _i64, _i64, _i64, _i64, _i64, _i64, _i, _p, _p],
    "rga3_gemm_lnq_bf16": [_p, _p, _p, _p, _p, _i64, _i64, _f, _p, _i64, _i64, _i64, _i64, _i64, _i64, _i, _i, _p],
    "rga3_rope_inplace": [_p, _p, _p, _i64, _i, _i, _i, _i64, _i64, _p],
    "rga3_gather_rows": [_p, _p, _p, _i64, _i64, _i64, _i64, _i64, _p],
    "rga3_scatter_rows": [_p, _p, _p, _i64, _i64, _i64, _i64, _i64, _p],
    "rga3_pad_cols": [_p, _p, _i64, _i64, _i64, _i64, _p],
    "rga3_silu_mul": [_p, _p, _p, _i64, _p],
    "rga3_add": [_p, _p, _p, _i64, _p],
    "rga3_cross_entropy_rows": [_p, _i, _p, _p, _p, _i64, _i64, _i64, _f, _p],
    "rga3_im2col": [_p, _p, _i64, _i, _i, _i, _i, _i, _i, _i64, _p],
    "rga3_maxpool2x2_win": [_p, _p, _i64, _i, _i, _i64, _i64, _p],
    "rga3_upsample2x_add": [_p, _p, _p, _i64, _i, _i, _i, _p],
    "rga3_add_bcast": [_p, _p, _p, _i64, _i64, _i, _i64, _i64, _i64, _f, _p],
    "rga3_bilinear": [_p, _i, _p, _p, _i64, _i, _i, _i, _i, _p],
    "rga3_conv3x3s2": [_p, _i, _p, _p, _p, _i64, _i, _i, _i, _i, _f, _f, _p],
    "rga3_decimg_rows": [_p, _i64, _p, _i64, _i, _p, _p, _i, _p, _p, _p, _p, _p, _p, _f, _p, _p, _p, _p, _p, _i64, _p, _p, _i64, _i, _f, _i64, _p],
    "rga3_attn_fewq": [_p, _i64, _p, _i64, _i64, _p, _p, _p, _i64, _i, _i, _i, _i, _f, _p],
    "rga3_copy_many": [_p, _p, _p, _i, _p],
    "rga3_conv3x3s2_ln_gelu": [_p, _i, _p, _p, _p, _p, _f, _p, _i64, _i, _i, _i, _i, _f, _f, _p],
    "rga3_dwconv7x7": [_p, _p, _p, _p, _i64, _i, _i, _i, _p],
    "rga3_rope_axial_inplace": [_p, _p, _p, _i64, _i, _i, _i64, _p],
    "rga3_pixel_shuffle2x": [_p, _p, _p, _p, _i64, _i, _i, _i, _i, _p],
    "rga3_bce_dice_sums": [_p, _p, _p, _i64, _i64, _p],
    "rga3_bce_dice_sums_ws_floats": [_i64, _i64],
    "rga3_bce_dice_sums_det": [_p, _p, _p, _p, _i64, _i64, _i64, _p],
    "rga3_mask_jf_ws_bytes": [_i64, _i64, _i64],
    "rga3_mask_jf_counts": [_p, _p, _p, _p, _p, _i64, _i64, _i64, _i64, _i, _p],
    "rga3_stom_ws_bytes": [_i64, _i64, _i64],
    "rga3_stom_flow": [_p, _p, _p, _i64, _i64, _i, _p],
    "rga3_stom_shift_composite": [_p, _p, _p, _p, _i64, _i64, _i64, _i, _p],
    "rga3_stom_mask_composite": [_p, _p, _p, _p, _p, _p, _i64, _i64, _i64, _i64, _i64, _i, _p, _i, _p, _i, _p],
    "rga3_attn_varlen_bwd": [_p, _p, _p, _p, _p, _p, _p, _p, _p, _p, _p, _p, _i, _i, _i, _i64, _i, _i, _i, _p, _f, _i, _p, _i64, _p],
    "rga3_transpose16_many": [_p, _p, _i, _p],
    "rga3_hiera_mlp144": [_p, _p, _p, _p, _p, _p, _p, _i64, _f, _p],
    "rga3_hiera_mlp288_pack_bytes": [],
    "rga3_hiera_mlp288_pack": [_p, _p, _p, _p, _p, _p],
    "rga3_hiera_mlp288": [_p, _p, _p, _p, _i64, _f, _p],
    "rga3_mlp3_rows": [_p, _p, _i, _i64, _p],
    "rga3_sam_select_objptr": [_p, _p, _p, _i64, _i, _p, _p, _p, _p, _p, _p, _p, _p, _p, _p, _i64, _p],
    "rga3_memattn_cross_ws_floats": [_i64, _i],
    "rga3_memattn_cross": [_p, _p, _p, _p, _i64, _i64, _i64, _i64, _i64, _i64, _f, _i, _p, _p],
    "rga3_memlayer_rows": [_p, _i64, _i, _p, _p, _i, _p, _p, _p, _i64, _p, _i64, _p, _p, _f, _p, _i64, _p, _p, _i, _p, _i64, _p, _p, _i, _i, _i64, _p],
    "rga3_gemm_rows16_many": [_p, _p, _i, _p],
    "rga3_gemm_stream_k_timeouts": [_p],
    "rga3_gemm_timeout_counter_offset": [],
    "rga3_gemm_ragged_plan": [_i64, _i64, _i64, _i, _i, _p, _p],
    "rga3_gemm_tiles": [_i, _p, _p, _p, _i],
    "rga3_gemm_candidates": [_i, _i64, _i64, _i64, _i, _i, _i, _p, _i],
    "rga3_gemm_tn_slices": [_i64, _i64, _i64],
    "rga3_quant_fp8_rows": [_p, _p, _p, _i64, _i64, _i64, _i64, _p],
    "rga3_gemm_fp8": [_p, _p, _p, _p, _p, _p, _p, _i64, _i64, _i64, _i64, _i64, _i64, _i64, _p],
    "rga3_swiglu_fwd_quant_fp8": [_p, _p, _p, _i64, _i64, _p],
    "rga3_swiglu_bwd_quant_fp8": [_p, _p, _p, _p, _i64, _i64, _p],
    "rga3_im2col3x3s2": [_p, _p, _i64, _i, _i, _i, _p],
    "rga3_pil_bicubic_coeffs": [_i, _i, _p, _p, _i64, _p],
    "rga3_sam_preprocess_u8": [_p, _i64, _i, _i, _i, _i, _p, _p, _i, _p, _p, _i, _p, _p, _p, _p, _p, _p],
    "rga3_qwen_norm_lut": [_p, _p, _i, _p],
    "rga3_qwen_patchify_u8": [_p, _i64, _i, _i, _p, _p, _i, _i, _i, _i, _p],
    "rga3_rmsnorm_bwd": [_p, _p, _p, _p, _p, _i64, _i64, _f, _p],
    "rga3_dropout_bf16": [_p, _p, _i64, _f, _i64, _i, _p],
    "rga3_dropout_pair_bf16": [_p, _p, _p, _p, _i64, _f, _i64, _f, _i64, _i, _p],
    "rga3_swiglu_fwd": [_p, _p, _i64, _i64, _p],
    "rga3_swiglu_bwd": [_p, _p, _p, _i64, _i64, _p],
    "rga3_transpose16": [_p, _p, _i64, _i64, _i64, _i64, _p],
    "rga3_segment_sum_rows": [_p, _p, _p, _p, _i64, _i64, _i64, _p],
    "rga3_adamw_step": [_p, _p, _p, _p, _p, _i64, _f, _f, _f, _f, _f, _i, _f, _p],
    "rga3_sumsq_accum": [_p, _p, _i64, _p],
    "rga3_sumsq_det": [_p, _i64, _p, _i64, _p, _i, _p],
    "rga3_adamw_step_clip": [_p, _p, _p, _p, _p, _i64, _f, _f, _f, _f, _f, _i, _p, _f, _p],
    "rga3_adamw_step_clip_rows": [_p, _p, _p, _p, _p, _i64, _i64, _p, _f, _f, _f, _f, _i, _p, _f, _p],
    "rga3_scatter_add_rows": [_p, _p, _p, _i64, _i64, _i64, _i64, _f, _p],
    "rga3_layernorm_bwd_ws_floats": [_i64, _i64],
    "rga3_layernorm_bwd": [_p, _p, _p, _p, _p, _p, _i64, _i64, _f, _p, _i64, _p],
    "rga3_colsum_accum": [_p, _p, _i64, _i64, _i64, _p],
    "rga3_colsum_ws_floats": [_i64, _i64],
    "rga3_colsum": [_p, _p, _i64, _i64, _i64, _p, _i64, _p, _p],
    "rga3_act": [_p, _p, _p, _i64, _i, _p],
    "rga3_bilinear_bwd": [_p, _p, _p, _i64, _i, _i, _i, _i, _p],
    "rga3_mask_product": [_p, _p, _p, _i64, _i64, _i64, _i64, _p],
    "rga3_mask_product_bwd_ws_floats": [_i64, _i64, _i64, _i64],
    "rga3_mask_product_bwd": [_p, _p, _p, _p, _p, _i64, _i64, _i64, _i64, _p, _i64, _p],
    "rga3_pixel_shuffle2x_bwd": [_p, _p, _i64, _i, _i, _i, _p],
    "rga3_bce_dice_grad": [_p, _p, _p, _p, _i64, _i64, _f, _f, _p],
    "rga3_bce_dice_grad_dev": [_p, _p, _p, _p, _i64, _i64, _p, _p, _p],
}

_INT64_RESULTS = ("rga3_gemm_lnsum_slices", "rga3_hiera_mlp288_pack_bytes", "rga3_gemm_workspace_bytes", "rga3_memattn_cross_ws_floats", "rga3_gemm_timeout_counter_offset", "rga3_layernorm_bwd_ws_floats", "rga3_colsum_ws_floats", "rga3_mask_product_bwd_ws_floats", "rga3_bce_dice_sums_ws_floats", "rga3_mask_jf_ws_bytes", "rga3_stom_ws_bytes")

_lib = None


class Rga3Error(RuntimeError):
    pass


def load():
    global _lib
    if _lib is not None:
        return _lib
    if not os.path.exists(LIB_PATH):
        raise Rga3Error(
            f"{LIB_PATH} not found: the HIP extension is required (no fallback path). "
            "Run `make -C rga3-release_amd/csrc` or `python -c 'import __graft_entry__ as g; g.build()'`.")
    import torch

    _thip = os.path.join(os.path.dirname(torch.__file__), "lib", "libamdhip64.so")
    if os.path.exists(_thip):
        C.CDLL(_thip, mode=C.RTLD_GLOBAL)
    lib = C.CDLL(LIB_PATH)
    for name, argtypes in SIGNATURES.items():
        fn = getattr(lib, name)
        fn.argtypes = argtypes
        fn.restype = C.c_int64 if name in _INT64_RESULTS else C.c_int
    _lib = lib
    return lib


def last_error() -> str:
    buf = C.create_string_buffer(512)
    load().rga3_last_error(buf, 512)
    return buf.value.decode("utf-8", "replace")


_TILE_ENTRIES = ("plain", "shared", "ln", "lnsum", "cat_k", "cat_n")
_tiles = {}


def gemm_tiles(entry: str) -> dict:
    if entry not in _tiles:
        ids, bm, bn = ((C.c_int * 64)() for _ in range(3))
        n = load().rga3_gemm_tiles(_TILE_ENTRIES.index(entry), ids, bm, bn, 64)
        if not 0 < n <= 64:
            raise Rga3Error("rga3_gemm_tiles failed: " + last_error())
        _tiles[entry] = {ids[i]: bn[i] for i in range(n)}
    return _tiles[entry]


def gemm_candidates(entry: str, M: int, N: int, K: int, act: int = 0, out_dtype: int = 0, bias=False, residual=False, colscale=False) -> tuple:
    ids = (C.c_int * 64)()
    n = load().rga3_gemm_candidates(_TILE_ENTRIES.index(entry), M, N, K, act, out_dtype, bool(bias) | bool(residual) << 1 | bool(colscale) << 2, ids, 64)
    if not 0 <= n <= 64:
        raise Rga3Error("rga3_gemm_candidates failed: " + last_error())
    return tuple(ids[:n])


def gemm_tn_slices(M: int, N: int, K: int) -> int:
    n = load().rga3_gemm_tn_slices(M, N, K)
    if n < 1:
        raise Rga3Error("rga3_gemm_tn_slices failed: " + last_error())
    return n


def check(rc: int, what: str):
    if rc != 0:
        raise Rga3Error(f"{what} failed (rc={rc}): {last_error()}")
```

### rga3-release_amd/rga3/hip/ops.py

```python
from __future__ import annotations

import math

import torch

from . import lib as _lib
from . import tuner as _tuner

BF16, F32 = 0, 1
ACT = {"none": 0, "gelu": 1, "swiglu": 2, "relu": 3}


def _stream():
    return torch.cuda.current_stream().cuda_stream


def _ptr(t):
    return 0 if t is None else t.data_ptr()


def _need_cuda(*ts):
    for t in ts:
        if t is not None and not t.is_cuda:
            raise _lib.Rga3Error("rga3 HIP ops need device tensors (no CPU fallback on the product path)")
# ... 635 lines not shown


def copy_many(pairs):
    import ctypes
    todo = []
    for d, s in pairs:
        nb = d.numel() * d.element_size()
        if (d.is_cuda and s.is_cuda and d.is_contiguous() and s.is_contiguous() and d.dtype == s.dtype and d.numel() == s.numel() and nb > 0 and nb % 16 == 0
                and d.data_ptr() % 16 == 0 and s.data_ptr() % 16 == 0):
            todo.append((d.data_ptr(), s.data_ptr(), nb))
        else:
            d.copy_(s)
    for i0 in range(0, len(todo), 24):
        part = todo[i0:i0 + 24]
        n = len(part)
        dp, sp, nb = (ctypes.c_void_p * n)(*[p_[0] for p_ in part]), (ctypes.c_void_p * n)(*[p_[1] for p_ in part]), (ctypes.c_int64 * n)(*[p_[2] for p_ in part])
        _lib.check(_lib.load().rga3_copy_many(ctypes.cast(dp, ctypes.c_void_p), ctypes.cast(sp, ctypes.c_void_p), ctypes.cast(nb, ctypes.c_void_p), n, _stream()),
                   "copy_many")


def conv3x3s2_ln_gelu_ok(x, weight) -> bool:
    co, ci = weight.shape[0], weight.shape[1]
    return (x.dtype == torch.float32 and (ci, co) == (1, 4)) or (x.dtype == torch.bfloat16 and (ci, co) == (4, 16))


def conv3x3s2_ln_gelu(x, weight, bias, ln_w, ln_b, eps: float, F: int, H: int, W: int, sig_scale: float = 0.0, sig_bias: float = 0.0):
    _need_cuda(x, weight, bias, ln_w, ln_b)
    Cout, Cin = weight.shape[0], weight.shape[1]
    assert conv3x3s2_ln_gelu_ok(x, weight) and weight.dtype == torch.bfloat16 and weight.is_contiguous() and x.is_contiguous() and x.numel() == F * H * W * Cin
    y = torch.empty((F * (H // 2) * (W // 2), Cout), dtype=torch.bfloat16, device=x.device)
    _lib.check(_lib.load().rga3_conv3x3s2_ln_gelu(x.data_ptr(), F32 if x.dtype == torch.float32 else BF16, weight.data_ptr(), _ptr(bias), ln_w.data_ptr(), _ptr(ln_b),
                                                  float(eps), y.data_ptr(), F, H, W, Cin, Cout, float(sig_scale), float(sig_bias), _stream()), "conv3x3s2_ln_gelu")
    return y


def conv3x3s2(x, weight, bias, F: int, H: int, W: int, sig_scale: float = 0.0, sig_bias: float = 0.0):
    _need_cuda(x, weight, bias)
    Cout, Cin = weight.shape[0], weight.shape[1]
    assert weight.dtype == torch.bfloat16 and weight.is_contiguous() and x.is_contiguous() and x.numel() == F * H * W * Cin
    if x.dtype == torch.bfloat16 and Cin % 8 == 0 and Cin >= 16:
        key = (weight.data_ptr(), weight._version)
        wp = _conv_pack.get(key)
        if wp is None:
            if len(_conv_pack) > 64:
                _conv_pack.clear()
            wp = _conv_pack[key] = weight.detach().permute(0, 2, 3, 1).reshape(Cout, 9 * Cin).contiguous()
        cols = torch.empty((F * (H // 2) * (W // 2), 9 * Cin), dtype=torch.bfloat16, device=x.device)
        _lib.check(_lib.load().rga3_im2col3x3s2(x.data_ptr(), cols.data_ptr(), F, H, W, Cin, _stream()), "im2col3x3s2")
        return gemm(cols, wp, bias)
    y = torch.empty((F * (H // 2) * (W // 2), Cout), dtype=torch.bfloat16, device=x.device)
    rc = _lib.load().rga3_conv3x3s2(x.data_ptr(), F32 if x.dtype == torch.float32 else BF16, weight.data_ptr(), _ptr(bias), y.data_ptr(), F, H, W,
                                    Cin, Cout, float(sig_scale), float(sig_bias), _stream())
    _lib.check(rc, "conv3x3s2")
    return y


def dwconv7x7(x, weight, bias, F: int, H: int, W: int):
    _need_cuda(x, weight, bias)
    assert x.dtype == torch.bfloat16 and x.is_contiguous() and weight.is_contiguous()
    y = torch.empty_like(x)
    _lib.check(_lib.load().rga3_dwconv7x7(x.data_ptr(), weight.data_ptr(), _ptr(bias), y.data_ptr(), F, H, W, x.shape[1], _stream()), "dwconv7x7")
    return y


def rope_axial_(x, cos, sin, n_rope: int):
    _need_cuda(x, cos, sin)
    assert x.dtype == torch.bfloat16 and x.dim() == 2 and x.stride(1) == 1 and cos.dtype == torch.float32 and cos.is_contiguous() and sin.is_contiguous()
    assert cos.shape[1] * 2 == x.shape[1]
    _lib.check(_lib.load().rga3_rope_axial_inplace(x.data_ptr(), cos.data_ptr(), sin.data_ptr(), int(n_rope), cos.shape[0], x.shape[1], x.stride(0),
                                                  _stream()), "rope_axial")
    return x


def mlp3_rows(specs, B: int):
    import ctypes
    n = len(specs)
    assert 1 <= n <= 8
    ptrs, dims, outs, keep = (ctypes.c_void_p * (8 * n))(), (ctypes.c_int64 * (6 * n))(), [], []
    for i, sp in enumerate(specs):
        x, xs, (w0, b0, w1, b1, w2, b2), sig = sp[:4]
        _need_cuda(x, w0, b0, w1, b1, w2, b2)
        for t in (w0, w1, w2):
            assert t.dtype == torch.bfloat16 and t.is_contiguous()
        assert x.dtype == torch.bfloat16 and tuple(w1.shape) == (w0.shape[0], w0.shape[0]) and w2.shape[1] == w0.shape[0], (w0.shape, w1.shape, w2.shape)
        y = sp[4] if len(sp) > 4 and sp[4] is not None else torch.empty((B, w2.shape[0]), dtype=torch.bfloat16, device=x.device)
        assert y.dtype == torch.bfloat16 and tuple(y.shape) == (B, w2.shape[0]) and y.stride(1) == 1
        for j, t in enumerate((x, w0, b0, w1, b1, w2, b2, y)):
            ptrs[8 * i + j] = _ptr(t)
        for j, v in enumerate((int(xs), y.stride(0), w0.shape[1], w0.shape[0], w2.shape[0], 1 if sig else 0)):
            dims[6 * i + j] = v
        outs.append(y)
    _lib.check(_lib.load().rga3_mlp3_rows(ctypes.cast(ptrs, ctypes.c_void_p), ctypes.cast(dims, ctypes.c_void_p), n, int(B), _stream()), "mlp3_rows")
    return outs


def sam_select_objptr(iou, obj, toks, proj, no_obj_ptr):
    _need_cuda(iou, obj, toks, no_obj_ptr, *proj)
    B, _, C = toks.shape
    assert iou.dtype == obj.dtype == toks.dtype == torch.bfloat16 and iou.is_contiguous() and obj.is_contiguous() and toks.stride(2) == 1 and toks.stride(1) == C
    best = torch.empty((2, B), dtype=torch.int64, device=toks.device)
    sel = torch.empty(B, dtype=torch.int32, device=toks.device)
    ptr = torch.empty((B, C), dtype=torch.bfloat16, device=toks.device)
    w0, b0, w1, b1, w2, b2 = proj
    _lib.check(_lib.load().rga3_sam_select_objptr(iou.data_ptr(), obj.data_ptr(), toks.data_ptr(), toks.stride(0), C, w0.data_ptr(), _ptr(b0), w1.data_ptr(), _ptr(b1),
                                                  w2.data_ptr(), _ptr(b2), no_obj_ptr.data_ptr(), best.data_ptr(), sel.data_ptr(), ptr.data_ptr(), B, _stream()),
               "sam_select_objptr")
    return best[0], sel, best[1], ptr


_memattn_ws = {}


def memattn_cross(q, k, m, scale: float, nsplit: int = 0, partials: bool = False):
    _need_cuda(q, k, m)
    assert q.dtype == k.dtype == m.dtype == torch.bfloat16 and q.dim() == k.dim() == m.dim() == 2
    assert q.shape[1] == 256 and k.shape[1] == 256 and m.shape[1] == 64 and k.shape[0] == m.shape[0], (q.shape, k.shape, m.shape)
    assert q.stride(1) == 1 and k.stride(1) == 1 and m.stride(1) == 1
    Nq, Nk = q.shape[0], k.shape[0]
    if nsplit <= 0:
        nqb = (Nq + 255) // 256
        nsplit = max(1, min(32, 256 // nqb, (Nk + 63) // 64))
    L = _lib.load()
    n = int(L.rga3_memattn_cross_ws_floats(Nq, nsplit))
    if n < 0:
        raise _lib.Rga3Error("memattn_cross: bad workspace query")
    key = _ws_key(q.device)
    ws = _memattn_ws.get(key)
    if ws is None or ws.numel() < n:
        ws = _memattn_ws[key] = torch.empty(n, dtype=torch.float32, device=q.device)
    if partials:
        _lib.check(L.rga3_memattn_cross(q.data_ptr(), k.data_ptr(), m.data_ptr(), None, Nq, Nk, q.stride(0), k.stride(0), m.stride(0), 0,
                                        float(scale), int(nsplit), ws.data_ptr(), _stream()), "memattn_cross")
        return ws[:nsplit * Nq * 64], ws[nsplit * Nq * 64:nsplit * Nq * 66], nsplit
    out = torch.empty((Nq, 64), dtype=torch.bfloat16, device=q.device)
    _lib.check(L.rga3_memattn_cross(q.data_ptr(), k.data_ptr(), m.data_ptr(), out.data_ptr(), Nq, Nk, q.stride(0), k.stride(0), m.stride(0), out.stride(0),
                                    float(scale), int(nsplit), ws.data_ptr(), _stream()), "memattn_cross")
    return out


def memlayer_rows(res, ln, eps: float, a=None, partials=None, w1=None, b1=None, want_x=True, want_t=False, w2=None, b2=None, rope=None, rope_cols: int = 0):
    wln, bln = ln
    _need_cuda(res, wln, bln, a, w1, b1, w2, b2)
    assert res.dtype == torch.bfloat16 and res.dim() == 2 and res.shape[1] == 256 and res.stride(1) == 1
    M, dev = res.shape[0], res.device
    x = t = y = None
    K1, po, pml, ns = 0, None, None, 0
    if w1 is not None:
        assert w1.dtype == torch.bfloat16 and w1.is_contiguous() and w1.shape[0] == 256
        K1 = w1.shape[1]
        if partials is not None:
            po, pml, ns = partials
            assert a is None and K1 == 64 and po.numel() == ns * M * 64 and pml.numel() == ns * M * 2
        else:
            assert a is not None and a.dtype == torch.bfloat16 and tuple(a.shape) == (M, K1) and a.stride(1) == 1
        if want_x:
            x = torch.empty((M, 256), dtype=torch.bfloat16, device=dev)
    else:
        assert a is None and partials is None
    if want_t or w2 is None:
        t = torch.empty((M, 256), dtype=torch.bfloat16, device=dev)
    N2, cos, sin, nq = 0, None, None, 0
    if w2 is not None:
        assert w2.dtype == torch.bfloat16 and w2.is_contiguous() and w2.shape[1] == 256 and w2.shape[0] in (256, 768)
        N2 = w2.shape[0]
        y = torch.empty((M, N2), dtype=torch.bfloat16, device=dev)
        if rope_cols:
            cos, sin = rope
            assert cos.dtype == sin.dtype == torch.float32 and cos.is_contiguous() and sin.is_contiguous() and cos.shape[1] == 128 and cos.shape == sin.shape
            nq = cos.shape[0]
    _lib.check(_lib.load().rga3_memlayer_rows(_ptr(a), a.stride(0) if a is not None else 0, K1, _ptr(po), _ptr(pml), ns, _ptr(w1), _ptr(b1), res.data_ptr(), res.stride(0),
                                              _ptr(x), 256, wln.data_ptr(), _ptr(bln), float(eps), _ptr(t), 256, _ptr(w2), _ptr(b2), N2, _ptr(y), N2 if N2 else 0,
                                              _ptr(cos), _ptr(sin), int(rope_cols), nq, M, _stream()), "memlayer_rows")
    return x, t, y


def pixel_shuffle2x(g, bias, add, F: int, H: int, W: int, act: str = "none"):
    _need_cuda(g, bias, add)
    Co = g.shape[1] // 4
    assert g.dtype == torch.bfloat16 and g.is_contiguous()
    out = torch.empty((F * 4 * H * W, Co), dtype=torch.bfloat16, device=g.device)
    _lib.check(_lib.load().rga3_pixel_shuffle2x(g.data_ptr(), _ptr(bias), _ptr(add), out.data_ptr(), F, H, W, Co, 1 if act == "gelu" else 0, _stream()),
               "pixel_shuffle2x")
    return out


def bce_dice_sums(logits, targets):
    _need_cuda(logits, targets)
    assert logits.dtype == targets.dtype == torch.float32 and logits.is_contiguous() and targets.is_contiguous() and logits.shape == targets.shape
    n = logits.shape[0]
    out = torch.empty((n, 4), dtype=torch.float32, device=logits.device)
    if n == 0:
        return out
    L = _lib.load()
    hw = logits[0].numel()
    nws = int(L.rga3_bce_dice_sums_ws_floats(n, hw))
    ws = torch.empty(nws, dtype=torch.float32, device=logits.device)
    _lib.check(L.rga3_bce_dice_sums_det(logits.data_ptr(), targets.data_ptr(), out.data_ptr(), ws.data_ptr(), nws, n, hw, _stream()), "bce_dice_sums_det")
    return out


def mask_jf_counts(annotation, segmentation, void_pixels=None, radius=None):
    _need_cuda(annotation, segmentation, void_pixels)
    ts = [t for t in (segmentation, annotation, void_pixels) if t is not None]
    for t in ts:
        if t.dtype not in (torch.bool, torch.uint8):
            raise _lib.Rga3Error(f"mask_jf_counts: masks are bool or uint8, got {t.dtype}")
        if t.shape != annotation.shape or t.device != annotation.device:
            raise _lib.Rga3Error(f"mask_jf_counts: shapes / devices differ: {tuple(t.shape)} on {t.device} vs {tuple(annotation.shape)} on {annotation.device}")
    if annotation.dim() not in (2, 3):
        raise _lib.Rga3Error(f"mask_jf_counts: [T, h, w] or [h, w] masks, got {tuple(annotation.shape)}")
    h, w = annotation.shape[-2:]
    T = annotation.shape[0] if annotation.dim() == 3 else 1
    if radius is None:
        radius = math.ceil(0.008 * math.hypot(h, w))
    if int(radius) != radius:
        raise _lib.Rga3Error(f"mask_jf_counts: radius {radius} is not an integer")
    L = _lib.load()
    nws = int(L.rga3_mask_jf_ws_bytes(T, h, w))
    if nws < 0:
        raise _lib.Rga3Error("mask_jf_ws_bytes failed: " + _lib.last_error())
    seg, ann, vd = (None if t is None else t.contiguous() for t in (segmentation, annotation, void_pixels))
    out = torch.empty((T, 6), dtype=torch.int64, device=ann.device)
    ws = torch.empty(nws, dtype=torch.uint8, device=ann.device)
    _lib.check(L.rga3_mask_jf_counts(seg.data_ptr(), ann.data_ptr(), _ptr(vd), out.data_ptr(), ws.data_ptr(), nws, T, h, w, int(radius), _stream()), "mask_jf_counts")
    return out


STOM_MAX_POINTS = 16384
STOM_MAX_KERNEL = 128
_stom_ws = {}


def _stom_points(name, tracks, visibility, vip_frame_idx):
    _need_cuda(tracks, visibility)
    if tracks.dtype != torch.float32 or tracks.dim() != 3 or tracks.shape[2] != 2 or not tracks.is_contiguous():
        raise _lib.Rga3Error(f"{name}: tracks are contiguous float32 [T, N, 2], got {tracks.dtype} {tuple(tracks.shape)}")
    T, N = tracks.shape[:2]
    if visibility.dtype not in (torch.bool, torch.uint8) or tuple(visibility.shape) != (T, N) or not visibility.is_contiguous() or visibility.device != tracks.device:
        raise _lib.Rga3Error(f"{name}: visibility is contiguous bool [{T}, {N}] on {tracks.device}, got {visibility.dtype} {tuple(visibility.shape)} on {visibility.device}")
    if not 1 <= N <= STOM_MAX_POINTS:
        raise _lib.Rga3Error(f"{name}: {N} points per frame (1..{STOM_MAX_POINTS})")
    if not 0 <= vip_frame_idx < T:
        raise _lib.Rga3Error(f"{name}: vip_frame_idx {vip_frame_idx} outside [0, {T})")
    return T, N


def _stom_frames(name, frames, overlay):
    _need_cuda(frames, overlay)
    if frames.dtype != torch.uint8 or frames.dim() != 4 or frames.shape[3] != 3 or frames.shape[0] == 0 or not frames.is_contiguous():
        raise _lib.Rga3Error(f"{name}: frames are contiguous uint8 [T, H, W, 3], got {frames.dtype} {tuple(frames.shape)}")
    T, H, W, _ = frames.shape
    if overlay.dtype != torch.uint8 or tuple(overlay.shape) != (H, W, 4) or not overlay.is_contiguous() or overlay.device != frames.device:
        raise _lib.Rga3Error(f"{name}: the overlay is contiguous uint8 [{H}, {W}, 4] on {frames.device}, got {overlay.dtype} {tuple(overlay.shape)} on {overlay.device}")
    return T, H, W


def stom_flow(tracks, visibility, vip_frame_idx: int):
    T, N = _stom_points("stom_flow", tracks, visibility, vip_frame_idx)
    rec = torch.empty((T, 4), dtype=torch.int32, device=tracks.device)
    _lib.check(_lib.load().rga3_stom_flow(tracks.data_ptr(), visibility.data_ptr(), rec.data_ptr(), T, N, int(vip_frame_idx), _stream()), "stom_flow")
    return rec


def stom_shift_composite(frames, overlay, records, vip_frame_idx: int):
    T, H, W = _stom_frames("stom_shift_composite", frames, overlay)
    _need_cuda(records)
    if records.dtype != torch.int32 or tuple(records.shape) != (T, 4) or not records.is_contiguous() or records.device != frames.device:
        raise _lib.Rga3Error(f"stom_shift_composite: records are contiguous int32 [{T}, 4] on {frames.device}, got {records.dtype} {tuple(records.shape)}")
    if not 0 <= vip_frame_idx < T:
        raise _lib.Rga3Error(f"stom_shift_composite: vip_frame_idx {vip_frame_idx} outside [0, {T})")
    out = torch.empty_like(frames)
    _lib.check(_lib.load().rga3_stom_shift_composite(frames.data_ptr(), overlay.data_ptr(), records.data_ptr(), out.data_ptr(), T, H, W, int(vip_frame_idx), _stream()),
               "stom_shift_composite")
    return out


def stom_mask_composite(frames, overlay, tracks, visibility, vip_frame_idx: int, spans, ksize: int, half_widths, radius: int):
    import numpy as np

    T, H, W = _stom_frames("stom_mask_composite", frames, overlay)
    Tp, N = _stom_points("stom_mask_composite", tracks, visibility, vip_frame_idx)
    if Tp != T or tracks.device != frames.device:
        raise _lib.Rga3Error(f"stom_mask_composite: {Tp} frames of tracks on {tracks.device} for {T} frames on {frames.device}")
    if not 0 <= ksize <= STOM_MAX_KERNEL:
        raise _lib.Rga3Error(f"stom_mask_composite: structuring element of {ksize} (0..{STOM_MAX_KERNEL})")
    spans = np.ascontiguousarray(spans, dtype=np.uint8)
    half_widths = np.ascontiguousarray(half_widths, dtype=np.uint8)
    if spans.shape != (max(ksize, 1), 2) or radius < 0 or half_widths.shape != (radius + 1,):
        raise _lib.Rga3Error(f"stom_mask_composite: spans {spans.shape} / half widths {half_widths.shape} do not fit ksize {ksize} / radius {radius}")
    L = _lib.load()
    nws = int(L.rga3_stom_ws_bytes(T, H, W))
    if nws < 0:
        raise _lib.Rga3Error("stom_ws_bytes failed: " + _lib.last_error())
    key = _ws_key(frames.device)
    ws = _stom_ws.get(key)
    if ws is None or ws.numel() < nws:
        ws = _stom_ws[key] = torch.empty(nws, dtype=torch.uint8, device=frames.device)
    out = torch.empty_like(frames)
    _lib.check(L.rga3_stom_mask_composite(frames.data_ptr(), overlay.data_ptr(), tracks.data_ptr(), visibility.data_ptr(), out.data_ptr(), ws.data_ptr(), nws, T, H, W, N,
                                          int(vip_frame_idx), spans.ctypes.data, int(ksize), half_widths.ctypes.data, int(radius), _stream()), "stom_mask_composite")
    return out


def attn_varlen_bwd(q, k, v, o, dout, lse, cu_q, cu_k, max_q: int, max_k: int, scale: float, causal: bool, dq=None, dk=None, dv=None):
    import ctypes
    _need_cuda(q, k, v, o, dout, lse)
    Tq, Hq, D = q.shape
    Hkv = k.shape[1]
    dq = torch.empty_like(q) if dq is None else dq
    dk = torch.empty((k.shape[0], Hkv, D), dtype=torch.bfloat16, device=q.device) if dk is None else dk
    dv = torch.empty((k.shape[0], Hkv, D), dtype=torch.bfloat16, device=q.device) if dv is None else dv
    for t in (q, k, v, o, dout, dq, dk, dv):
        assert t.dtype == torch.bfloat16 and t.stride(2) == 1
    delta = torch.empty((Hq, Tq), dtype=torch.float32, device=q.device)
    Tk = k.shape[0]
    dkv_ws = torch.empty((2 * Hq * Tk * D,), dtype=torch.float32, device=q.device) if (Hq > Hkv and D % 4 == 0) else None
    st = (ctypes.c_int64 * 16)(q.stride(0), q.stride(1), k.stride(0), k.stride(1), v.stride(0), v.stride(1), o.stride(0), o.stride(1),
                               dout.stride(0), dout.stride(1), dq.stride(0), dq.stride(1), dk.stride(0), dk.stride(1), dv.stride(0), dv.stride(1))
    rc = _lib.load().rga3_attn_varlen_bwd(q.data_ptr(), k.data_ptr(), v.data_ptr(), o.data_ptr(), dout.data_ptr(), lse.data_ptr(), dq.data_ptr(),
                                          dk.data_ptr(), dv.data_ptr(), delta.data_ptr(), cu_q.data_ptr(), cu_k.data_ptr(), cu_q.numel() - 1, int(max_q),
                                          int(max_k), Tq, Hq, Hkv, D, ctypes.cast(st, ctypes.c_void_p), float(scale), int(bool(causal)), _ptr(dkv_ws), Tk, _stream())
    _lib.check(rc, "attn_varlen_bwd")
    return dq, dk, dv


def rmsnorm_bwd(x, weight, dy, eps: float, add=None):
    _need_cuda(x, weight, dy, add)
    assert x.is_contiguous() and dy.is_contiguous() and x.dtype == dy.dtype == torch.bfloat16 and (add is None or add.is_contiguous())
    dx = torch.empty_like(x)
    _lib.check(_lib.load().rga3_rmsnorm_bwd(x.data_ptr(), weight.data_ptr(), dy.data_ptr(), _ptr(add), dx.data_ptr(), x.shape[0], x.shape[1], float(eps),
                                            _stream()), "rmsnorm_bwd")
    return dx


def quant_fp8_rows(x):
    _need_cuda(x)
    assert x.dtype == torch.bfloat16 and x.dim() == 2 and x.stride(1) == 1 and x.shape[1] % 8 == 0
    rows, K = x.shape
    q = torch.empty((rows, K), dtype=torch.uint8, device=x.device)
    sc = torch.empty((rows,), dtype=torch.float32, device=x.device)
    _lib.check(_lib.load().rga3_quant_fp8_rows(x.data_ptr(), q.data_ptr(), sc.data_ptr(), rows, K, x.stride(0), q.stride(0), _stream()), "quant_fp8_rows")
    return q, sc


def gemm_fp8(aq, sa, wq, sw, bias=None, residual=None, out=None):
    _need_cuda(aq, wq, sa, sw, bias, residual)
    assert aq.dtype == torch.uint8 and wq.dtype == torch.uint8 and aq.stride(1) == 1 and wq.stride(1) == 1 and aq.shape[1] == wq.shape[1]
    M, K = aq.shape
    N = wq.shape[0]
    if out is None:
        out = torch.empty((M, N), dtype=torch.bfloat16, device=aq.device)
    assert out.dtype == torch.bfloat16 and out.stride(1) == 1 and sa.dtype == torch.float32 and sw.dtype == torch.float32
    _lib.check(_lib.load().rga3_gemm_fp8(aq.data_ptr(), wq.data_ptr(), sa.data_ptr(), sw.data_ptr(), _ptr(bias), _ptr(residual), out.data_ptr(), M, N, K,
                                         aq.stride(0), wq.stride(0), out.stride(0), residual.stride(0) if residual is not None else 0, _stream()), "gemm_fp8")
    return out


def swiglu_fwd_quant(gu):
    _need_cuda(gu)
    assert gu.dtype == torch.bfloat16 and gu.is_contiguous() and gu.shape[1] % 32 == 0
    T, I = gu.shape[0], gu.shape[1] // 2
    q = torch.empty((T, I), dtype=torch.uint8, device=gu.device)
    sc = torch.empty((T,), dtype=torch.float32, device=gu.device)
    _lib.check(_lib.load().rga3_swiglu_fwd_quant_fp8(gu.data_ptr(), q.data_ptr(), sc.data_ptr(), T, I, _stream()), "swiglu_fwd_quant_fp8")
    return q, sc


def swiglu_bwd_quant(gu, da):
    _need_cuda(gu, da)
    assert gu.dtype == da.dtype == torch.bfloat16 and gu.is_contiguous() and da.is_contiguous() and gu.shape[1] == 2 * da.shape[1]
    T, I = da.shape
    q = torch.empty((T, 2 * I), dtype=torch.uint8, device=gu.device)
    sc = torch.empty((T,), dtype=torch.float32, device=gu.device)
    _lib.check(_lib.load().rga3_swiglu_bwd_quant_fp8(gu.data_ptr(), da.data_ptr(), q.data_ptr(), sc.data_ptr(), T, I, _stream()), "swiglu_bwd_quant_fp8")
    return q, sc


def dropout(x, p: float, seed: int, out=None, accumulate: bool = False):
    _need_cuda(x, out)
    assert x.dtype == torch.bfloat16 and x.is_contiguous() and x.numel() % 8 == 0
    if out is None:
        assert not accumulate
        out = torch.empty_like(x)
    assert out.is_contiguous() and out.shape == x.shape and out.dtype == torch.bfloat16
    _lib.check(_lib.load().rga3_dropout_bf16(x.data_ptr(), out.data_ptr(), x.numel(), float(p), int(seed) & 0x7FFFFFFFFFFFFFFF, int(bool(accumulate)), _stream()),
               "dropout")
    return out


def dropout_pair(xa, pa: float, seed_a: int, xb, pb: float, seed_b: int, accumulate_into=None):
    _need_cuda(xa, xb, accumulate_into)
    assert xa.dtype == xb.dtype == torch.bfloat16 and xa.is_contiguous() and xb.is_contiguous() and xa.shape == xb.shape and xa.numel() % 8 == 0
    L = _lib.load()
    if accumulate_into is None:
        ya, yb = torch.empty_like(xa), torch.empty_like(xb)
        _lib.check(L.rga3_dropout_pair_bf16(xa.data_ptr(), xb.data_ptr(), ya.data_ptr(), yb.data_ptr(), xa.numel(), float(pa), int(seed_a), float(pb), int(seed_b), 0,
                                            _stream()), "dropout_pair_bf16")
        return ya, yb
    out = accumulate_into
    assert out.dtype == torch.bfloat16 and out.is_contiguous() and out.shape == xa.shape
    _lib.check(L.rga3_dropout_pair_bf16(xa.data_ptr(), xb.data_ptr(), out.data_ptr(), None, xa.numel(), float(pa), int(seed_a), float(pb), int(seed_b), 1, _stream()),
               "dropout_pair_bf16")
    return out


def swiglu_fwd(gu):
    _need_cuda(gu)
    assert gu.dtype == torch.bfloat16 and gu.is_contiguous() and gu.shape[1] % 32 == 0
    a = torch.empty((gu.shape[0], gu.shape[1] // 2), dtype=torch.bfloat16, device=gu.device)
    _lib.check(_lib.load().rga3_swiglu_fwd(gu.data_ptr(), a.data_ptr(), gu.shape[0], gu.shape[1] // 2, _stream()), "swiglu_fwd")
    return a


def swiglu_bwd(gu, da):
    _need_cuda(gu, da)
    assert gu.is_contiguous() and da.is_contiguous() and gu.shape[1] == 2 * da.shape[1]
    dgu = torch.empty_like(gu)
    _lib.check(_lib.load().rga3_swiglu_bwd(gu.data_ptr(), da.data_ptr(), dgu.data_ptr(), gu.shape[0], da.shape[1], _stream()), "swiglu_bwd")
    return dgu


def transpose(x):
    _need_cuda(x)
    assert x.dim() == 2 and x.stride(1) == 1 and x.element_size() == 2
    R, C = x.shape
    out = torch.empty((C, R), dtype=x.dtype, device=x.device)
    _lib.check(_lib.load().rga3_transpose16(x.data_ptr(), out.data_ptr(), R, C, x.stride(0), R, _stream()), "transpose16")
    return out


def transpose_many(mats):
    import ctypes
    outs = []
    for a in range(0, len(mats), 64):
        grp = mats[a:a + 64]
        n = len(grp)
        ptrs, dims = (ctypes.c_void_p * (2 * n))(), (ctypes.c_int64 * (2 * n))()
        for i, x in enumerate(grp):
            _need_cuda(x)
            assert x.dim() == 2 and x.is_contiguous() and x.element_size() == 2
            o = torch.empty((x.shape[1], x.shape[0]), dtype=x.dtype, device=x.device)
            ptrs[2 * i], ptrs[2 * i + 1] = x.data_ptr(), o.data_ptr()
            dims[2 * i], dims[2 * i + 1] = x.shape[0], x.shape[1]
            outs.append(o)
        _lib.check(_lib.load().rga3_transpose16_many(ctypes.cast(ptrs, ctypes.c_void_p), ctypes.cast(dims, ctypes.c_void_p), n, _stream()), "transpose16_many")
    return outs


def segment_sum_rows(x, rows, offsets):
    _need_cuda(x, rows, offsets)
    assert x.dtype == torch.bfloat16 and x.stride(1) == 1 and rows.dtype == torch.int64 and offsets.dtype == torch.int64
    n = offsets.numel() - 1
    out = torch.empty((n, x.shape[1]), dtype=torch.bfloat16, device=x.device)
    if n > 0:
        _lib.check(_lib.load().rga3_segment_sum_rows(x.data_ptr(), rows.data_ptr(), offsets.data_ptr(), out.data_ptr(), n, x.shape[1], x.stride(0), _stream()),
                   "segment_sum_rows")
    return out


def adamw_step_(param, master, grad, m, v, lr, beta1, beta2, eps, weight_decay, step: int, grad_scale: float = 1.0):
    _need_cuda(param, master, grad, m, v)
    assert param.dtype == grad.dtype == torch.bfloat16 and master.dtype == m.dtype == v.dtype == torch.float32
    assert param.is_contiguous() and grad.is_contiguous() and master.is_contiguous()
    _lib.check(_lib.load().rga3_adamw_step(param.data_ptr(), master.data_ptr(), grad.data_ptr(), m.data_ptr(), v.data_ptr(), param.numel(), float(lr),
                                           float(beta1), float(beta2), float(eps), float(weight_decay), int(step), float(grad_scale), _stream()), "adamw_step")


def sumsq_accum_(g, out):
    _need_cuda(g, out)
    assert g.dtype == torch.bfloat16 and g.is_contiguous() and out.dtype == torch.float32
    _lib.check(_lib.load().rga3_sumsq_accum(g.data_ptr(), out.data_ptr(), g.numel(), _stream()), "sumsq_accum")


def sumsq_det_(g, partials, out, accumulate: bool):
    _need_cuda(g, partials, out)
    assert g.dtype == torch.bfloat16 and g.is_contiguous() and out.dtype == partials.dtype == torch.float32
    _lib.check(_lib.load().rga3_sumsq_det(g.data_ptr(), g.numel(), partials.data_ptr(), partials.numel(), out.data_ptr(), int(bool(accumulate)), _stream()), "sumsq_det")


def adamw_step_clip_(param, master, grad, m, v, lr, beta1, beta2, eps, weight_decay, step: int, sumsq=None, max_norm: float = 0.0):
    _need_cuda(param, master, grad, m, v, sumsq)
    assert param.dtype == grad.dtype == torch.bfloat16 and master.dtype == m.dtype == v.dtype == torch.float32
    assert param.is_contiguous() and grad.is_contiguous() and master.is_contiguous()
    _lib.check(_lib.load().rga3_adamw_step_clip(param.data_ptr(), master.data_ptr(), grad.data_ptr(), m.data_ptr(), v.data_ptr(), param.numel(), float(lr),
                                                float(beta1), float(beta2), float(eps), float(weight_decay), int(step), _ptr(sumsq), float(max_norm), _stream()),
               "adamw_step_clip")


def adamw_step_clip_rows_(param, master, grad, m, v, row_active, lr, beta1, beta2, eps, step: int, sumsq=None, max_norm: float = 0.0):
    _need_cuda(param, master, grad, m, v, row_active, sumsq)
    assert param.dtype == grad.dtype == torch.bfloat16 and master.dtype == m.dtype == v.dtype == torch.float32 and row_active.dtype == torch.uint8
    assert param.dim() == 2 and param.is_contiguous() and grad.is_contiguous() and master.is_contiguous() and row_active.numel() == param.shape[0]
    _lib.check(_lib.load().rga3_adamw_step_clip_rows(param.data_ptr(), master.data_ptr(), grad.data_ptr(), m.data_ptr(), v.data_ptr(), param.shape[0], param.shape[1],
                                                     row_active.data_ptr(), float(lr), float(beta1), float(beta2), float(eps), int(step), _ptr(sumsq), float(max_norm),
                                                     _stream()), "adamw_step_clip_rows")


def scatter_add_rows_(dst, idx, src, scale: float = 1.0):
    _need_cuda(dst, idx, src)
    assert dst.dtype == src.dtype == torch.bfloat16 and idx.dtype == torch.int64 and dst.dim() == 2 and src.dim() == 2
    assert dst.stride(1) == 1 and src.stride(1) == 1 and dst.shape[1] == src.shape[1] and idx.numel() == src.shape[0]
    if idx.numel():
        _lib.check(_lib.load().rga3_scatter_add_rows(dst.data_ptr(), idx.data_ptr(), src.data_ptr(), idx.numel(), dst.shape[1], dst.stride(0), src.stride(0),
                                                     float(scale), _stream()), "scatter_add_rows")
    return dst


def check_gemm_health(device=None):
    n = gemm_stream_k_timeouts(device)
    if n:
        for t in _gemm_ws.values():
            t[:4096].zero_()
        raise _lib.Rga3Error(f"stream-K GEMM hand-off timed out {n} time(s): results since the last check are not trustworthy (workspace flags re-zeroed)")


class GemmHealthWatch:

    def __init__(self, every: int = 16):
        self.every, self.n, self.pending = max(1, int(every)), 0, []

    def poll(self):
        self.n += 1
        if self.n % self.every:
            return
        self.examine()
        for (dev, _), t in _gemm_ws.items():
            with torch.cuda.device(dev):
                off = int(_lib.load().rga3_gemm_timeout_counter_offset())
                if off < 0:
                    continue
                host = torch.empty(1, dtype=torch.int32).pin_memory()
                host.copy_(t[off:off + 4].view(torch.int32), non_blocking=True)
                ev = torch.cuda.Event()
                ev.record()
            self.pending.append((host, ev))

    def examine(self):
        pend, self.pending = self.pending, []
        for host, ev in pend:
            ev.synchronize()
            if int(host[0]) != 0:
                for t in _gemm_ws.values():
                    t[:4096].zero_()
                raise _lib.Rga3Error(f"stream-K GEMM hand-off timed out {int(host[0])} time(s) in the last {2 * self.every} optimizer steps: their results are not "
                                     "trustworthy (workspace flags re-zeroed)")


_inference_watch = GemmHealthWatch(every=1)


def poll_gemm_health():
    if _gemm_ws:
        _inference_watch.poll()


def layernorm_bwd(x, weight, dy, eps: float, want_param_grads=True):
    _need_cuda(x, weight, dy)
    assert x.is_contiguous() and dy.is_contiguous() and x.dtype == dy.dtype == torch.bfloat16
    L = _lib.load()
    dx = torch.empty_like(x)
    dw = db = ws = None
    nws = 0
    if want_param_grads:
        nws = int(L.rga3_layernorm_bwd_ws_floats(x.shape[0], x.shape[1]))
        if nws:
            dw = torch.empty(x.shape[1], dtype=torch.float32, device=x.device)
            db = torch.empty(x.shape[1], dtype=torch.float32, device=x.device)
            ws = torch.empty(nws, dtype=torch.float32, device=x.device)
        else:
            dw = torch.zeros(x.shape[1], dtype=torch.float32, device=x.device)
            db = torch.zeros(x.shape[1], dtype=torch.float32, device=x.device)
    _lib.check(L.rga3_layernorm_bwd(x.data_ptr(), weight.data_ptr(), dy.data_ptr(), dx.data_ptr(), _ptr(dw), _ptr(db), x.shape[0], x.shape[1],
                                    float(eps), _ptr(ws), nws, _stream()), "layernorm_bwd")
    return dx, dw, db


def colsum(x, fused_finish: bool = False):
    _need_cuda(x)
    assert x.dtype == torch.bfloat16 and x.dim() == 2 and x.stride(1) == 1
    L = _lib.load()
    rows, cols = x.shape
    if cols % 8 == 0 and x.stride(0) % 8 == 0 and x.data_ptr() % 16 == 0:
        nws = int(L.rga3_colsum_ws_floats(rows, cols))
        out = torch.empty(cols, dtype=torch.float32, device=x.device)
        ws = torch.empty(nws, dtype=torch.float32, device=x.device)
        _lib.check(L.rga3_colsum(x.data_ptr(), out.data_ptr(), rows, cols, x.stride(0), ws.data_ptr(), nws,
                                 _tn_counters(x.device)[128:].data_ptr() if fused_finish else None, _stream()), "colsum")
        return out
    out = torch.zeros(cols, dtype=torch.float32, device=x.device)
    _lib.check(L.rga3_colsum_accum(x.data_ptr(), out.data_ptr(), rows, cols, x.stride(0), _stream()), "colsum_accum")
    return out


def mask_product(hyper, up, P: int):
    _need_cuda(hyper, up)
    assert hyper.dtype == up.dtype == torch.bfloat16 and hyper.is_contiguous() and up.is_contiguous() and hyper.dim() == 3 and up.dim() == 2
    B, NM, C = hyper.shape
    assert up.shape == (B * P, C)
    masks = torch.empty((B, NM, P), dtype=torch.float32, device=up.device)
    _lib.check(_lib.load().rga3_mask_product(hyper.data_ptr(), up.data_ptr(), masks.data_ptr(), B, NM, P, C, _stream()), "mask_product")
    return masks


def mask_product_bwd(dmasks, hyper, up, P: int):
    _need_cuda(dmasks, hyper, up)
    assert dmasks.dtype == torch.float32 and dmasks.is_contiguous() and hyper.is_contiguous() and up.is_contiguous()
    B, NM, C = hyper.shape
    L = _lib.load()
    nws = int(L.rga3_mask_product_bwd_ws_floats(B, NM, P, C))
    ws = torch.empty(nws, dtype=torch.float32, device=up.device)
    dup = torch.empty_like(up)
    dhyper = torch.empty_like(hyper)
    _lib.check(L.rga3_mask_product_bwd(dmasks.data_ptr(), hyper.data_ptr(), up.data_ptr(), dup.data_ptr(), dhyper.data_ptr(), B, NM, P, C, ws.data_ptr(), nws,
                                       _stream()), "mask_product_bwd")
    return dhyper, dup


def gelu(x):
    _need_cuda(x)
    assert x.dtype == torch.bfloat16 and x.is_contiguous()
    out = torch.empty_like(x)
    _lib.check(_lib.load().rga3_act(x.data_ptr(), 0, out.data_ptr(), x.numel(), 0, _stream()), "act")
    return out


def act_bwd(a, dy, kind: str):
    _need_cuda(a, dy)
    assert a.dtype == dy.dtype == torch.bfloat16 and a.is_contiguous() and dy.is_contiguous()
    out = torch.empty_like(a)
    _lib.check(_lib.load().rga3_act(a.data_ptr(), dy.data_ptr(), out.data_ptr(), a.numel(), 1 if kind == "gelu" else 2, _stream()), "act")
    return out
# ... 33 lines not shown
```

### rga3-release_amd/rga3/model/qwen_train.py

```python
from __future__ import annotations

import math
import os

import numpy as np
import torch
import torch.nn as nn

from ..hip import ops
from ..utils.staging import upload
from . import qwen2_5_vl as _Q
from .qwen2_5_vl import GatedMLP, Linear, _versions


class LoRALinear(Linear):

    def __init__(self, base: Linear, r: int, alpha: float, dropout: float = 0.0):
        super().__init__(base.in_features, base.out_features, bias=base.bias is not None, device=base.weight.device, dtype=base.weight.dtype)
        self.weight, self.bias = base.weight, base.bias
        self.weight.requires_grad_(False)
        if self.bias is not None:
            self.bias.requires_grad_(False)
        mk = lambda i, o: Linear(i, o, bias=False, device=base.weight.device, dtype=base.weight.dtype)
        self.lora_A = nn.ModuleDict({"default": mk(base.in_features, r)})
# ... 109 lines not shown
    if isinstance(lin, LoRALinear):
        return lin.lora_A["default"].weight, lin.lora_B["default"].weight, lin.scaling
    return None


_lora_cache = {}


def _lora_versions(lin):
    A, B = lin.lora_A["default"].weight, lin.lora_B["default"].weight
    return A._version, A.data_ptr(), B._version, B.data_ptr()


def _lora_build(mods):
    groups = {}
    for m in mods:
        A, B = m.lora_A["default"].weight, m.lora_B["default"].weight
        groups.setdefault((tuple(A.shape), tuple(B.shape), float(m.scaling), A.dtype, A.device), []).append(m)
    with torch.no_grad():
        for (_, _, sc, _, _), grp in groups.items():
            A = torch.stack([m.lora_A["default"].weight.detach() for m in grp])
            B = torch.stack([m.lora_B["default"].weight.detach() for m in grp])
            As = A * sc
            At = A.transpose(1, 2).contiguous()
            Bts = (B * sc).transpose(1, 2).contiguous()
            for i, m in enumerate(grp):
                _lora_cache[id(m)] = (_lora_versions(m), As[i], At[i], Bts[i])


def lora_refresh(layers):
    mods = [p for layer in layers for p in (layer.self_attn.q_proj, layer.self_attn.v_proj) if isinstance(p, LoRALinear)]
    if mods and any((e := _lora_cache.get(id(m))) is None or e[0] != _lora_versions(m) for m in (mods[0], mods[-1])):
        _lora_build(mods)
    ats = [layer.self_attn for layer in layers if _lora_cat_ok(layer.self_attn)]
    if ats and len({(a.num_heads, a.num_kv, a.head_dim, a.q_proj.lora_A["default"].weight.shape[0], float(a.q_proj.scaling), float(a.v_proj.scaling)) for a in ats}) == 1:
        if any((e := _lora_cat.get(id(a))) is None or e[0] != _lora_versions(a.q_proj) + _lora_versions(a.v_proj) for a in (ats[0], ats[-1])):
            _lora_cat_build(ats)


_LORA_FOLD = os.environ.get("RGA3_LORA_FOLD", "1") != "0"
_SWIGLU_PRE = os.environ.get("RGA3_SWIGLU_PRE", "1") != "0"
_lora_cat = {}
_lora_cat_store = {}


def set_lora_fold(on: bool):
    global _LORA_FOLD
    _LORA_FOLD = bool(on)


def _lora_cat_ok(at) -> bool:
    q, v = at.q_proj, at.v_proj
    if not (_LORA_FOLD and isinstance(q, LoRALinear) and isinstance(v, LoRALinear)) or isinstance(at.k_proj, LoRALinear):
        return False
    rq, rv = q.lora_A["default"].weight.shape[0], v.lora_A["default"].weight.shape[0]
    return rq == rv and (2 * rq) % 64 == 0 and q.lora_A["default"].weight.dtype == torch.bfloat16 and q.weight.shape[1] % 64 == 0


def _lora_cat_build(ats):
    with torch.no_grad():
        at0 = ats[0]
        Hq, Hk, D = at0.num_heads, at0.num_kv, at0.head_dim
        r = at0.q_proj.lora_A["default"].weight.shape[0]
        Nq, Nall = Hq * D, (Hq + 2 * Hk) * D
        Bq = torch.stack([a.q_proj.lora_B["default"].weight.detach() for a in ats])
        Bv = torch.stack([a.v_proj.lora_B["default"].weight.detach() for a in ats])
        ids = tuple(id(a) for a in ats)
        key = (ids, Nall, r, Bq.dtype, Bq.device)
        st = _lora_cat_store.get(key)
        if st is None:
            for k in [k for k in _lora_cat_store if k != key and not set(k[0]).isdisjoint(ids)]:
                del _lora_cat_store[k]
            st = (torch.zeros((len(ats), Nall, 2 * r), dtype=Bq.dtype, device=Bq.device), torch.zeros((len(ats), 2 * r, Nall), dtype=Bq.dtype, device=Bq.device))
            _lora_cat_store[key] = st
        W2, Wn = st
        W2[:, :Nq, :r] = Bq
        W2[:, Nq + Hk * D:, r:] = Bv
        Wn[:, :r, :Nq] = (Bq * float(at0.q_proj.scaling)).transpose(1, 2)
        Wn[:, r:, Nq + Hk * D:] = (Bv * float(at0.v_proj.scaling)).transpose(1, 2)
        for i, a in enumerate(ats):
            _lora_cat[id(a)] = (_lora_versions(a.q_proj) + _lora_versions(a.v_proj), W2[i], Wn[i])


def _lora_cat_ops(at):
    e = _lora_cat.get(id(at))
    if e is None or e[0] != _lora_versions(at.q_proj) + _lora_versions(at.v_proj):
        _lora_cat_build([at])
        e = _lora_cat[id(at)]
    return e[1], e[2]


def _lora_ops(lin):
    e = _lora_cache.get(id(lin))
    if e is None or e[0] != _lora_versions(lin):
        _lora_build([lin])
        e = _lora_cache[id(lin)]
    return e[1], e[2], e[3]


_drop_state = {"step": 0}


def next_dropout_seed(layer_idx: int, which: int, advance: bool = True) -> int:
    if advance:
        _drop_state["step"] += 1
    base = torch.initial_seed() & 0xFFFFFF
    return ((base << 39) ^ (_drop_state["step"] << 12) ^ (layer_idx << 2) ^ which) & 0x7FFFFFFFFFFFFFFF


def preview_dropout_seeds(n_layers: int):
    saved = _drop_state["step"]
    try:
        return [(next_dropout_seed(li, 0), next_dropout_seed(li, 1, advance=False)) for li in range(n_layers)]
    finally:
        _drop_state["step"] = saved


def _lora_dropout(at):
    pq = at.q_proj.dropout_p if isinstance(at.q_proj, LoRALinear) and at.q_proj.training else 0.0
    pv = at.v_proj.dropout_p if isinstance(at.v_proj, LoRALinear) and at.v_proj.training else 0.0
    return pq, pv


def _drop_pair(h1, pq, pv, seeds):
    if pq > 0.0 and pv > 0.0 and h1.is_contiguous():
        return ops.dropout_pair(h1, pq, seeds[0], h1, pv, seeds[1])
    return (ops.dropout(h1, pq, seeds[0]) if pq > 0.0 else h1), (ops.dropout(h1, pv, seeds[1]) if pv > 0.0 else h1)


def qkv_with_lora(at, h1, seeds=None, want_inputs=False):
    Hq, Hk, D = at.num_heads, at.num_kv, at.head_dim
    wqkv, bqkv = at._packed()
    lq, lv = _lora_parts(at.q_proj), _lora_parts(at.v_proj)
    pq, pv = _lora_dropout(at)
    if seeds is None and (pq > 0.0 or pv > 0.0):
        lid = getattr(at, "layer_idx", 0) or 0
        seeds = (next_dropout_seed(lid, 0), next_dropout_seed(lid, 1, advance=False))
    if not _fp8["on"] and h1.shape[0] > 16 and _lora_cat_ok(at):
        r = lq[0].shape[0]
        hq, hv = _drop_pair(h1, pq, pv, seeds)
        tt = torch.empty((h1.shape[0], 2 * r), dtype=h1.dtype, device=h1.device)
        tq = ops.gemm(hq, _lora_ops(at.q_proj)[0], out=tt[:, :r])
        tv = ops.gemm(hv, _lora_ops(at.v_proj)[0], out=tt[:, r:])
        qkv2 = ops.gemm_cat(h1, wqkv, bqkv, a2=tt, w2=_lora_cat_ops(at)[0])
        return (qkv2, tq, tv, hq, hv) if want_inputs else (qkv2, tq, tv)
    if _fp8["on"] and h1.shape[1] % 128 == 0:
        qkv2 = _fgemm(h1, at, "wqkv", (at.q_proj.weight, at.k_proj.weight, at.v_proj.weight), lambda: wqkv, bias=bqkv)
    else:
        qkv2 = ops.gemm(h1, wqkv, bqkv)
    tq = tv = None
    hq = hv = h1
    if lq is not None and lv is not None and pq > 0.0 and pv > 0.0:
        hq, hv = _drop_pair(h1, pq, pv, seeds)
        pq = pv = 0.0
    if lq is not None:
        if pq > 0.0:
            hq = ops.dropout(h1, pq, seeds[0])
        tq = ops.gemm(hq, _lora_ops(at.q_proj)[0])
        oq = qkv2[:, : Hq * D]
        ops.gemm(tq, lq[1].detach(), residual=oq, out=oq)
    if lv is not None:
        if pv > 0.0:
            hv = ops.dropout(h1, pv, seeds[1])
        tv = ops.gemm(hv, _lora_ops(at.v_proj)[0])
        ov = qkv2[:, (Hq + Hk) * D:]
        ops.gemm(tv, lv[1].detach(), residual=ov, out=ov)
    return (qkv2, tq, tv, hq, hv) if want_inputs else (qkv2, tq, tv)


def _layer_forward_fp8(layer, x, cos, sin, cu, max_len, seeds):
    at, mlp = layer.self_attn, layer.mlp
    Hq, Hk, D = at.num_heads, at.num_kv, at.head_dim
    T = x.shape[0]
    w1, w2 = layer.input_layernorm, layer.post_attention_layernorm
    h1 = ops.rmsnorm(x, w1.weight, w1.variance_epsilon)
    qkv2 = qkv_with_lora(at, h1, seeds=seeds)[0]
    qkv = qkv2.view(T, Hq + 2 * Hk, D)
    ops.rope_(qkv, cos, sin, 0, Hq + Hk)
    att = ops.attn_varlen(qkv[:, :Hq], qkv[:, Hq:Hq + Hk], qkv[:, Hq + Hk:], cu, cu, max_len, D ** -0.5, causal=True)
    x1 = _fgemm(att.view(T, Hq * D), at, "wo", (at.o_proj.weight,), lambda: at.o_proj.weight.detach(), residual=x)
    h2 = ops.rmsnorm(x1, w2.weight, w2.variance_epsilon)
    wgu, bgu, wd = mlp._packed()
    gu = _fgemm(h2, mlp, "wgu", (mlp.gate_proj.weight, mlp.up_proj.weight), lambda: wgu, bias=bgu)
    return _down_from_gu(mlp, gu, wd, x1)


def _down_from_gu(mlp, gu, wd, x1):
    if _fp8_fused(gu.shape[1] // 2):
        aq, asc = ops.swiglu_fwd_quant(gu)
        return _fgemm_q(aq, asc, mlp, "wd", (mlp.down_proj.weight,), lambda: wd, bias=mlp.down_proj.bias, residual=x1)
    return _fgemm(ops.swiglu_fwd(gu), mlp, "wd", (mlp.down_proj.weight,), lambda: wd, bias=mlp.down_proj.bias, residual=x1)


_acts = {"store": True}


def set_activation_recompute(on: bool):
    _acts["store"] = not on


def _layer_forward_store(layer, x, cos, sin, cu, max_len, seeds):
    at, mlp = layer.self_attn, layer.mlp
    Hq, Hk, D = at.num_heads, at.num_kv, at.head_dim
    T = x.shape[0]
    w1, w2 = layer.input_layernorm, layer.post_attention_layernorm
    h1 = ops.rmsnorm(x, w1.weight, w1.variance_epsilon)
    qkv2, tq, tv, hq_in, hv_in = qkv_with_lora(at, h1, seeds=seeds, want_inputs=True)
    qkv = qkv2.view(T, Hq + 2 * Hk, D)
    ops.rope_(qkv, cos, sin, 0, Hq + Hk)
    att, lse = ops.attn_varlen(qkv[:, :Hq], qkv[:, Hq:Hq + Hk], qkv[:, Hq + Hk:], cu, cu, max_len, D ** -0.5, causal=True, return_lse=True)
    x1 = _fgemm(att.view(T, Hq * D), at, "wo", (at.o_proj.weight,), lambda: at.o_proj.weight.detach(), residual=x)
    h2 = ops.rmsnorm(x1, w2.weight, w2.variance_epsilon)
    wgu, bgu, wd = mlp._packed()
    if not _fp8["on"] and _SWIGLU_PRE and T > 4:
        a_, gu = ops.gemm_swiglu_pre(h2, wgu, bgu)
        y = _fgemm(a_, mlp, "wd", (mlp.down_proj.weight,), lambda: wd, bias=mlp.down_proj.bias, residual=x1)
    else:
        gu = _fgemm(h2, mlp, "wgu", (mlp.gate_proj.weight, mlp.up_proj.weight), lambda: wgu, bias=bgu)
        y = _down_from_gu(mlp, gu, wd, x1)
    return y, (h1, qkv, att, lse, x1, h2, gu, tq, tv, hq_in, hv_in)


_neg = {}


def _neg_table(sin):
    key = (sin.data_ptr(), sin._version, tuple(sin.shape))
    if _neg.get("key") != key:
        _neg["key"], _neg["t"] = key, (-sin).contiguous()
        _neg["src"] = sin
    return _neg["t"]


class DecoderLayerFn(torch.autograd.Function):

    @staticmethod
    def forward(ctx, x, aq, bq, av, bv, layer, cos, sin, cu, max_len, seeds):
        at0 = layer.self_attn
        ctx.stored = False
        if _acts["store"]:
            with torch.no_grad():
                y, saved = _layer_forward_store(layer, x, cos, sin, cu, max_len, seeds)
            ctx.stored = True
            ctx.seeds = seeds
            ctx.layer, ctx.cos, ctx.sin, ctx.cu, ctx.max_len = layer, cos, sin, cu, max_len
            ctx.save_for_backward(x, *saved)
            return y
        if _fp8["on"]:
            with torch.no_grad():
                y = _layer_forward_fp8(layer, x, cos, sin, cu, max_len, seeds)
        else:
            at0._lora_drop_seeds = seeds
            try:
                with torch.no_grad():
                    y = layer(x, cos, sin, cu, max_len, None)
            finally:
                at0._lora_drop_seeds = None
        ctx.seeds = seeds
        ctx.layer, ctx.cos, ctx.sin, ctx.cu, ctx.max_len = layer, cos, sin, cu, max_len
        ctx.save_for_backward(x)
        return y

    @staticmethod
    def backward(ctx, dy):
        x = ctx.saved_tensors[0]
        layer, cos, sin, cu, max_len = ctx.layer, ctx.cos, ctx.sin, ctx.cu, ctx.max_len
        at, mlp = layer.self_attn, layer.mlp
        Hq, Hk, D = at.num_heads, at.num_kv, at.head_dim
        T = x.shape[0]
        dy = dy.contiguous()
        with torch.no_grad():
            w1, w2 = layer.input_layernorm, layer.post_attention_layernorm
            wqkv, bqkv = at._packed()
            lq, lv = _lora_parts(at.q_proj), _lora_parts(at.v_proj)
            pq, pv = _lora_dropout(at)
            wgu, bgu, wd = mlp._packed()
            if ctx.stored:
                h1, qkv, att, lse, x1, h2, gu, tq, tv, hq_in, hv_in = ctx.saved_tensors[1:]
            else:
                h1 = ops.rmsnorm(x, w1.weight, w1.variance_epsilon)
                qkv2, tq, tv, hq_in, hv_in = qkv_with_lora(at, h1, seeds=ctx.seeds, want_inputs=True)
                qkv = qkv2.view(T, Hq + 2 * Hk, D)
                ops.rope_(qkv, cos, sin, 0, Hq + Hk)
                att, lse = ops.attn_varlen(qkv[:, :Hq], qkv[:, Hq:Hq + Hk], qkv[:, Hq + Hk:], cu, cu, max_len, D ** -0.5, causal=True, return_lse=True)
                x1 = _fgemm(att.view(T, Hq * D), at, "wo", (at.o_proj.weight,), lambda: at.o_proj.weight.detach(), residual=x)
                h2 = ops.rmsnorm(x1, w2.weight, w2.variance_epsilon)
                gu = _fgemm(h2, mlp, "wgu", (mlp.gate_proj.weight, mlp.up_proj.weight), lambda: wgu, bias=bgu)
            q, k, v = qkv[:, :Hq], qkv[:, Hq:Hq + Hk], qkv[:, Hq + Hk:]
            da = _fgemm(dy, mlp, "wd_t", (mlp.down_proj.weight,), lambda: ops.transpose(wd))
            if _fp8_fused(gu.shape[1]):
                dq, dsc = ops.swiglu_bwd_quant(gu, da)
                del gu, da
                dh2 = _fgemm_q(dq, dsc, mlp, "wgu_t", (mlp.gate_proj.weight, mlp.up_proj.weight), lambda: ops.transpose(wgu))
                del dq
            else:
                dgu = ops.swiglu_bwd(gu, da)
                del gu, da
                dh2 = _fgemm(dgu, mlp, "wgu_t", (mlp.gate_proj.weight, mlp.up_proj.weight), lambda: ops.transpose(wgu))
                del dgu
            dx1 = ops.rmsnorm_bwd(x1, w2.weight, dh2, w2.variance_epsilon, add=dy)
            datt = _fgemm(dx1, at, "wo_t", (at.o_proj.weight,), lambda: ops.transpose(at.o_proj.weight.detach())).view(T, Hq, D)
            dqkv = torch.empty_like(qkv)
            ops.attn_varlen_bwd(q, k, v, att, datt, lse, cu, cu, max_len, max_len, D ** -0.5, True, dq=dqkv[:, :Hq], dk=dqkv[:, Hq:Hq + Hk],
                                dv=dqkv[:, Hq + Hk:])
            ops.rope_(dqkv, cos, _neg_table(sin), 0, Hq + Hk)
            dqkv2 = dqkv.view(T, (Hq + 2 * Hk) * D)
            fold = (not _fp8["on"]) and T > 16 and _lora_cat_ok(at)
            dtt = None
            if fold:
                wqkv_t = _wt(at, "wqkv_t", at.q_proj.weight, at.k_proj.weight, at.v_proj.weight, build=lambda: ops.transpose(wqkv))
                dh1, dtt = ops.gemm_cat(dqkv2, wqkv_t, wn=_lora_cat_ops(at)[1])
            else:
                dh1 = _fgemm(dqkv2, at, "wqkv_t", (at.q_proj.weight, at.k_proj.weight, at.v_proj.weight), lambda: ops.transpose(wqkv))
            grads = [None, None, None, None]
            if lq is not None or lv is not None:
                tn_pairs, tn_slots = [], []
                pend = []
                for slot, lp, lin, t_, cols, pdrop, hin, sd in ((0, lq, at.q_proj, tq, (0, Hq * D), pq, hq_in, 0),
                                                                (2, lv, at.v_proj, tv, ((Hq + Hk) * D, (Hq + 2 * Hk) * D), pv, hv_in, 1)):
                    if lp is None:
                        continue
                    _, At, Bts = _lora_ops(lin)
                    dsl = dqkv2[:, cols[0]:cols[1]]
                    if dtt is not None:
                        rr = dtt.shape[1] // 2
                        dt = dtt[:, :rr] if slot == 0 else dtt[:, rr:]
                    else:
                        dt = ops.gemm(dsl, Bts)
                    tn_pairs += [(dt, h1 if pdrop == 0.0 else hin), (dsl, t_)]
                    tn_slots += [slot, slot + 1]
                    if pdrop == 0.0:
                        ops.gemm(dt, At, residual=dh1, out=dh1)
                    else:
                        pend.append((ops.gemm(dt, At), pdrop, ctx.seeds[sd]))
                if len(pend) == 2 and dh1.is_contiguous():
                    ops.dropout_pair(pend[0][0], pend[0][1], pend[0][2], pend[1][0], pend[1][1], pend[1][2], accumulate_into=dh1)
                else:
                    for xg, pg, sg in pend:
                        ops.dropout(xg, pg, sg, out=dh1, accumulate=True)
                for sl, gw in zip(tn_slots, ops.gemm_tn_many(tn_pairs)):
                    grads[sl] = gw
            dx = ops.rmsnorm_bwd(x, w1.weight, dh1, w1.variance_epsilon, add=dx1)
        return (dx, grads[0], grads[1], grads[2], grads[3], None, None, None, None, None, None)


class EmbedFn(torch.autograd.Function):

    @staticmethod
    def forward(ctx, weight, ids_dev, ids_np, grad_rows_np, plan=None):
        from ..parallel.ddp import sparse_sink_for

        ctx.shape = weight.shape
        ctx.sink = sparse_sink_for(weight)
        ctx.weight = weight
        plan = plan if plan is not None else {}
        if "embed_bwd" not in plan:
            rows = grad_rows_np
            ids = ids_np[rows]
            order = np.argsort(ids, kind="stable")
            uniq, counts = np.unique(ids[order], return_counts=True)
            off = np.concatenate([[0], np.cumsum(counts)]).astype(np.int64)
            dev = weight.device
            plan["embed_bwd"] = (upload(rows[order].astype(np.int64), dev), upload(off, dev), upload(uniq.astype(np.int64), dev),
                                 uniq.astype(np.int64))
        ctx.csr = plan["embed_bwd"]
        if ctx.sink is not None:
            ctx.sink.announce_sparse(weight, ctx.csr[3])
        return ops.gather_rows(weight, ids_dev)

    @staticmethod
    def backward(ctx, dx):
        rows_dev, off_dev, uniq_dev, _ = ctx.csr
        seg = ops.segment_sum_rows(dx.contiguous(), rows_dev, off_dev)
        if ctx.sink is not None:
            ctx.sink.add_sparse(ctx.weight, uniq_dev, seg)
            return None, None, None, None, None
        dW = torch.zeros(ctx.shape, dtype=dx.dtype, device=dx.device)
        ops.scatter_rows_(dW, uniq_dev, seg)
        return dW, None, None, None, None


class NormHeadCEFn(torch.autograd.Function):

    @staticmethod
    def forward(ctx, h, lm_w, norm_w, eps, valid_rows_dev, targets_dev, n_valid):
        hn = ops.rmsnorm(h, norm_w, eps)
        if n_valid == 0:
            ctx.n = 0
            ctx.save_for_backward(h, norm_w)
            ctx.eps = eps
            return torch.zeros((), device=h.device, dtype=torch.float32), hn
        hv = ops.gather_rows(hn, valid_rows_dev)
        logits = ops.gemm(hv, lm_w)
        row_loss, dlogits = ops.cross_entropy_rows(logits, targets_dev, want_grad=True, grad_scale=1.0 / n_valid)
        ctx.save_for_backward(h, lm_w, norm_w, hv, dlogits, valid_rows_dev)
        ctx.eps, ctx.n = eps, n_valid
        return row_loss.sum() / n_valid, hn

    @staticmethod
    def backward(ctx, gloss, ghn):
        if ctx.n == 0:
            h, norm_w = ctx.saved_tensors
            with torch.no_grad():
                dh = ops.rmsnorm_bwd(h, norm_w, ghn.contiguous() if ghn is not None else torch.zeros_like(h), ctx.eps)
            return dh, None, None, None, None, None, None
        h, lm_w, norm_w, hv, dlogits, rows = ctx.saved_tensors
        n = ctx.n
        with torch.no_grad():
            dlogits = (dlogits.float() * gloss).to(dlogits.dtype)
            dW = None
            if lm_w.requires_grad:
                from ..parallel.ddp import dense_grad_out_for
                dW = ops.gemm_tn(dlogits, hv, out=dense_grad_out_for(lm_w))
            n8 = (n + 7) // 8 * 8
            dl = dlogits
            if n8 != n:
                dl = torch.zeros((n8, dlogits.shape[1]), dtype=dlogits.dtype, device=dlogits.device)
                dl[:n] = dlogits
            dhv = ops.gemm_tn(ops.transpose(dl), lm_w.detach())[:n].contiguous()
            dhn = ghn.contiguous().clone() if ghn is not None else torch.zeros_like(h)
            dhn_rows = ops.add(ops.gather_rows(dhn, rows), dhv)
            ops.scatter_rows_(dhn, rows, dhn_rows)
            dh = ops.rmsnorm_bwd(h, norm_w, dhn, ctx.eps)
        return dh, dW, None, None, None, None, None


def lm_train_forward(model, x, pos3, cu, max_len, labels_np, am_cur, flat_keep, lens, plan=None):
    tm = model.model
    cos, sin = tm.mrope_tables(pos3)
    lora_refresh(tm.layers)
    for li, layer in enumerate(tm.layers):
        at = layer.self_attn
        lq, lv = _lora_parts(at.q_proj), _lora_parts(at.v_proj)
        pq, pv = _lora_dropout(at)
        seeds = (next_dropout_seed(li, 0), next_dropout_seed(li, 1, advance=False)) if (pq > 0.0 or pv > 0.0) else None
        x = DecoderLayerFn.apply(x, lq[0] if lq else None, lq[1] if lq else None, lv[0] if lv else None, lv[1] if lv else None, layer, cos, sin,
                                 cu, max_len, seeds)
    plan = plan if plan is not None else {}
    if "train_targets" not in plan:
        B, S = labels_np.shape
        nxt = np.full((B, S), -100, dtype=np.int64)
        nxt[:, :-1] = labels_np[:, 1:]
        tgt = nxt.reshape(-1)[flat_keep]
        valid = np.flatnonzero(tgt != -100)
        dev = x.device
        plan["train_targets"] = (upload(valid.astype(np.int64), dev), upload(tgt[valid], dev), int(valid.size))
    valid_dev, tgt_dev, n_valid = plan["train_targets"]
    loss, hn = NormHeadCEFn.apply(x, model.lm_head.weight, tm.norm.weight, tm.norm.variance_epsilon, valid_dev, tgt_dev, n_valid)
    return loss, hn
```

Before: 7.551.

## Fuse RoPE backward into attention bwd epilogues and dropout-pair into rmsnorm bwd

Applies the inverse rotary rotation to dq inside the dq kernel epilogue and to dk inside a new GQA dK/dV reduce kernel, replacing a separate rope_ pass over dqkv. It also folds the two LoRA dropout-gradient accumulations into the rmsnorm backward kernel, so dh1 is no longer read and written by a standalone dropout_pair kernel. This removes two memory-bound elementwise passes per decoder layer in the backward pass. The cost is extra register pressure and cos/sin loads in the attention epilogue, plus dropout hashing in the rmsnorm kernel.

```diff
diff --git a/include/rga3_hip.h b/include/rga3_hip.h
--- a/include/rga3_hip.h
+++ b/include/rga3_hip.h
@@ -120,6 +120,10 @@
                          void* dk, void* dv, float* delta_ws, const int32_t* cu_q, const int32_t* cu_k, int nseg, int max_q,
                          int max_k, int64_t total_q, int Hq, int Hkv, int D, const int64_t* strides16, float scale, int causal,
                          float* dkv_ws, int64_t total_k, void* stream);
+int rga3_attn_varlen_bwd_rope(const void* q, const void* k, const void* v, const void* o, const void* dout, const float* lse, void* dq,
+                              void* dk, void* dv, float* delta_ws, const int32_t* cu_q, const int32_t* cu_k, int nseg, int max_q,
+                              int max_k, int64_t total_q, int Hq, int Hkv, int D, const int64_t* strides16, float scale, int causal,
+                              float* dkv_ws, int64_t total_k, const float* cos, const float* sin, void* stream);
 int rga3_hiera_mlp144(const void* x, const void* w1f, const float* c1, const void* d1, const void* w2, const void* b2, void* y, int64_t M, float eps, void* stream);
 int64_t rga3_hiera_mlp288_pack_bytes(void);
 int rga3_hiera_mlp288_pack(const void* w1f, const float* c1, const void* d1, const void* w2, void* pack, void* stream);
@@ -143,6 +147,8 @@
 int rga3_gemm_tn_slices(int64_t M, int64_t N, int64_t K);
 int rga3_rmsnorm_bwd(const void* x, const void* weight, const void* dy, const void* add, void* dx, int64_t rows, int64_t dim, float eps,
                      void* stream);
+int rga3_rmsnorm_bwd_drop2(const void* x, const void* weight, const void* dy, const void* add, void* dx, int64_t rows, int64_t dim, float eps,
+                           const void* ga, const void* gb, float pa, int64_t seed_a, float pb, int64_t seed_b, void* stream);
 int rga3_dropout_bf16(const void* x, void* y, int64_t n, float p, int64_t seed, int accumulate, void* stream);
 int rga3_dropout_pair_bf16(const void* xa, const void* xb, void* ya, void* yb, int64_t n, float pa, int64_t seed_a, float pb, int64_t seed_b, int sum, void* stream);
 int rga3_swiglu_fwd(const void* gu, void* a, int64_t T, int64_t I, void* stream);
diff --git a/rga3-release_amd/csrc/attn_bwd.hip b/rga3-release_amd/csrc/attn_bwd.hip
--- a/rga3-release_amd/csrc/attn_bwd.hip
+++ b/rga3-release_amd/csrc/attn_bwd.hip
@@ -16,11 +16,26 @@
     float* dkv_ws;
     long total_k;
     int gx, gy;
+    const float *rope_cos = nullptr, *rope_sin = nullptr;
 };
 
+__device__ __forceinline__ void rope_quad(u32x2& a, u32x2& b, const float* cs, const float* sn, int d, int half) {
+    const f32x4 c1 = *(const f32x4*)(cs + d), s1 = *(const f32x4*)(sn + d), c2 = *(const f32x4*)(cs + d + half), s2 = *(const f32x4*)(sn + d + half);
+    float o1[4], o2[4];
+#pragma unroll
+    for (int e = 0; e < 4; ++e) {
+        const float x = (e & 1) ? __uint_as_float(a[e >> 1] & 0xffff0000u) : __uint_as_float(a[e >> 1] << 16);
+        const float y = (e & 1) ? __uint_as_float(b[e >> 1] & 0xffff0000u) : __uint_as_float(b[e >> 1] << 16);
+        o1[e] = __builtin_fmaf(x, c1[e], -(y * s1[e]));
+        o2[e] = __builtin_fmaf(y, c2[e], x * s2[e]);
+    }
+    a[0] = pack_bf2(o1[0], o1[1]); a[1] = pack_bf2(o1[2], o1[3]);
+    b[0] = pack_bf2(o2[0], o2[1]); b[1] = pack_bf2(o2[2], o2[3]);
+}
+
 constexpr int BT = 64;
 
-template <int DP, int QT, int NWAVE, bool PAIR>
+template <int DP, int QT, int NWAVE, bool PAIR, bool ROPE = false>
 __global__ __launch_bounds__(64 * NWAVE) void attn_bwd_dq_kernel(AttnBwdArgs p) {
     constexpr int NT = 64 * NWAVE;
     constexpr int BLOCK_M = NWAVE * QT * 16;
@@ -202,6 +217,23 @@
         const int qi = qw0 + t * 16 + c;
         if (qi < Lq) {
             unsigned short* row = p.dq + (long)(qs + qi) * p.dq_st + (long)hq * p.dq_sh;
+            if constexpr (ROPE) {
+                const float* cs = p.rope_cos + (long)(qs + qi) * DP;
+                const float* sn = p.rope_sin + (long)(qs + qi) * DP;
+#pragma unroll
+                for (int d = 0; d < DT / 2; ++d) {
+                    const int dd = d * 16 + 4 * g;
+                    u32x2 a, b;
+                    a[0] = pack_bf2(dqacc[t][d][0], dqacc[t][d][1]);
+                    a[1] = pack_bf2(dqacc[t][d][2], dqacc[t][d][3]);
+                    b[0] = pack_bf2(dqacc[t][d + DT / 2][0], dqacc[t][d + DT / 2][1]);
+                    b[1] = pack_bf2(dqacc[t][d + DT / 2][2], dqacc[t][d + DT / 2][3]);
+                    rope_quad(a, b, cs, sn, dd, DP / 2);
+                    *(u32x2*)(row + dd) = a;
+                    *(u32x2*)(row + dd + DP / 2) = b;
+                }
+                continue;
+            }
 #pragma unroll
             for (int d = 0; d < DT; ++d) {
                 const int dd = d * 16 + 4 * g;
@@ -433,6 +465,39 @@
     *(u32x2*)(p.dv + key * p.dv_st + (long)hk * p.dv_sh + dd) = b;
 }
 
+__global__ __launch_bounds__(256) void attn_dkv_reduce_rope_kernel(AttnBwdArgs p) {
+    const int group = p.Hq / p.Hkv;
+    const int half = p.D / 2, d8 = p.D / 8;
+    const long idx = (long)blockIdx.x * 256 + threadIdx.x;
+    const long total = p.total_k * p.Hkv * d8;
+    if (idx >= total) return;
+    const int dd = (int)(idx % d8) * 4;
+    const long row = idx / d8;
+    const int hk = (int)(row % p.Hkv);
+    const long key = row / p.Hkv;
+    const long plane = p.total_k * p.Hkv * (long)p.D, hf = (long)group * plane;
+    const float* w = p.dkv_ws + row * p.D + dd;
+    f32x4 sk1 = *(const f32x4*)w, sk2 = *(const f32x4*)(w + half), sv1 = *(const f32x4*)(w + hf), sv2 = *(const f32x4*)(w + hf + half);
+    for (int h = 1; h < group; ++h) {
+        sk1 += *(const f32x4*)(w + h * plane);
+        sk2 += *(const f32x4*)(w + h * plane + half);
+        sv1 += *(const f32x4*)(w + hf + h * plane);
+        sv2 += *(const f32x4*)(w + hf + h * plane + half);
+    }
+    u32x2 a, b, c, d;
+    a[0] = pack_bf2(sk1[0], sk1[1]); a[1] = pack_bf2(sk1[2], sk1[3]);
+    b[0] = pack_bf2(sk2[0], sk2[1]); b[1] = pack_bf2(sk2[2], sk2[3]);
+    c[0] = pack_bf2(sv1[0], sv1[1]); c[1] = pack_bf2(sv1[2], sv1[3]);
+    d[0] = pack_bf2(sv2[0], sv2[1]); d[1] = pack_bf2(sv2[2], sv2[3]);
+    rope_quad(a, b, p.rope_cos + key * p.D, p.rope_sin + key * p.D, dd, half);
+    unsigned short* rk = p.dk + key * p.dk_st + (long)hk * p.dk_sh + dd;
+    unsigned short* rv = p.dv + key * p.dv_st + (long)hk * p.dv_sh + dd;
+    *(u32x2*)rk = a;
+    *(u32x2*)(rk + half) = b;
+    *(u32x2*)rv = c;
+    *(u32x2*)(rv + half) = d;
+}
+
 template <auto K>
 static int launch_bwd_grid(AttnBwdArgs& a, int lds, unsigned gx, int gy, int nseg, int nwave, hipStream_t st, const char* name) {
     a.gx = (int)gx; a.gy = gy;
@@ -455,6 +520,19 @@
     const unsigned nqb = (unsigned)cdiv(max_q, BLOCK_M), nkb = (unsigned)cdiv(max_k, 16 * NW);
     const bool pair = a.causal && nqb >= 4 && nkb >= 4;
     const unsigned gq = pair ? (nqb + 1) / 2 : nqb, gk = pair ? (nkb + 1) / 2 : nkb;
+    if constexpr (DP % 32 == 0) {
+        if (a.rope_cos) {
+            if (int rc = pair ? launch_bwd_grid<attn_bwd_dq_kernel<DP, QT, NWQ, true, true>>(a, LDS_DQ, gq, a.Hq, nseg, NWQ, st, "attn_bwd_dq_kernel<rope>")
+                              : launch_bwd_grid<attn_bwd_dq_kernel<DP, QT, NWQ, false, true>>(a, LDS_DQ, gq, a.Hq, nseg, NWQ, st, "attn_bwd_dq_kernel<rope>"))
+                return rc;
+            if (int rc = pair ? launch_bwd_grid<attn_bwd_dkv_kernel<DP, NW, true, true>>(a, LDS_DKV, gk, a.Hq, nseg, NW, st, "attn_bwd_dkv_kernel<split>")
+                              : launch_bwd_grid<attn_bwd_dkv_kernel<DP, NW, true, false>>(a, LDS_DKV, gk, a.Hq, nseg, NW, st, "attn_bwd_dkv_kernel<split>"))
+                return rc;
+            hipLaunchKernelGGL(attn_dkv_reduce_rope_kernel, dim3((unsigned)cdiv(a.total_k * a.Hkv * (a.D / 8), 256)), dim3(256), 0, st, a);
+            RGA3_CHECK_LAUNCH("attn_dkv_reduce_rope_kernel");
+            return 0;
+        }
+    }
     if (int rc = pair ? launch_bwd_grid<attn_bwd_dq_kernel<DP, QT, NWQ, true>>(a, LDS_DQ, gq, a.Hq, nseg, NWQ, st, "attn_bwd_dq_kernel")
                       : launch_bwd_grid<attn_bwd_dq_kernel<DP, QT, NWQ, false>>(a, LDS_DQ, gq, a.Hq, nseg, NWQ, st, "attn_bwd_dq_kernel"))
         return rc;
@@ -475,10 +553,10 @@
 
 using namespace rga3;
 
-extern "C" int rga3_attn_varlen_bwd(const void* q, const void* k, const void* v, const void* o, const void* dout, const float* lse,
-                                    void* dq, void* dk, void* dv, float* delta_ws, const int32_t* cu_q, const int32_t* cu_k, int nseg,
-                                    int max_q, int max_k, int64_t total_q, int Hq, int Hkv, int D, const int64_t* strides16, float scale,
-                                    int causal, float* dkv_ws, int64_t total_k, void* stream) {
+static int attn_varlen_bwd_impl(const void* q, const void* k, const void* v, const void* o, const void* dout, const float* lse,
+                               void* dq, void* dk, void* dv, float* delta_ws, const int32_t* cu_q, const int32_t* cu_k, int nseg,
+                               int max_q, int max_k, int64_t total_q, int Hq, int Hkv, int D, const int64_t* strides16, float scale,
+                               int causal, float* dkv_ws, int64_t total_k, const float* cos, const float* sin, void* stream) {
     RGA3_CHECK_ARG(q && k && v && o && dout && lse && dq && dk && dv && delta_ws && cu_q && cu_k && strides16, "attn_bwd: null pointer");
     RGA3_CHECK_ARG(nseg > 0 && max_q > 0 && max_k > 0 && total_q > 0, "attn_bwd: sizes");
     RGA3_CHECK_ARG(Hq > 0 && Hkv > 0 && Hq % Hkv == 0, "attn_bwd: Hq=%d Hkv=%d", Hq, Hkv);
@@ -502,9 +580,33 @@
     a.Hq = Hq; a.Hkv = Hkv; a.D = D; a.total_q = total_q; a.scale = scale; a.scale_log2 = scale * 1.4426950408889634f; a.causal = causal;
     a.dkv_ws = dkv_ws; a.total_k = total_k;
     RGA3_CHECK_ARG(!dkv_ws || (total_k > 0 && D % 4 == 0), "attn_bwd: dkv_ws needs total_k");
+    RGA3_CHECK_ARG(!cos == !sin, "attn_bwd: cos and sin go together");
+    if (cos) {
+        RGA3_CHECK_ARG(D % 32 == 0 && dkv_ws && Hq > Hkv, "attn_bwd: the rotation of dq / dk takes D %% 32 == 0 and the split dK / dV path (Hq > Hkv with a workspace)");
+        RGA3_CHECK_ARG((((uintptr_t)cos | (uintptr_t)sin) & 15) == 0, "attn_bwd: cos / sin tables must be 16-byte aligned");
+    }
+    a.rope_cos = cos; a.rope_sin = sin;
     hipStream_t st = (hipStream_t)stream;
     if (D <= 32) return launch_bwd<32>(a, nseg, max_q, max_k, st);
     if (D <= 64) return launch_bwd<64>(a, nseg, max_q, max_k, st);
     if (D <= 96) return launch_bwd<96>(a, nseg, max_q, max_k, st);
     return launch_bwd<128>(a, nseg, max_q, max_k, st);
 }
+
+extern "C" int rga3_attn_varlen_bwd(const void* q, const void* k, const void* v, const void* o, const void* dout, const float* lse,
+                                    void* dq, void* dk, void* dv, float* delta_ws, const int32_t* cu_q, const int32_t* cu_k, int nseg,
+                                    int max_q, int max_k, int64_t total_q, int Hq, int Hkv, int D, const int64_t* strides16, float scale,
+                                    int causal, float* dkv_ws, int64_t total_k, void* stream) {
+    return attn_varlen_bwd_impl(q, k, v, o, dout, lse, dq, dk, dv, delta_ws, cu_q, cu_k, nseg, max_q, max_k, total_q, Hq, Hkv, D, strides16, scale, causal, dkv_ws,
+                                total_k, nullptr, nullptr, stream);
+}
+
+extern "C" int rga3_attn_varlen_bwd_rope(const void* q, const void* k, const void* v, const void* o, const void* dout, const float* lse,
+                                         void* dq, void* dk, void* dv, float* delta_ws, const int32_t* cu_q, const int32_t* cu_k, int nseg,
+                                         int max_q, int max_k, int64_t total_q, int Hq, int Hkv, int D, const int64_t* strides16, float scale,
+                                         int causal, float* dkv_ws, int64_t total_k, const float* cos, const float* sin, void* stream) {
+    RGA3_CHECK_ARG(cos && sin, "attn_bwd_rope: null cos / sin table");
+    RGA3_CHECK_ARG(total_q == total_k, "attn_bwd_rope: one table row per token: total_q %ld != total_k %ld", (long)total_q, (long)total_k);
+    return attn_varlen_bwd_impl(q, k, v, o, dout, lse, dq, dk, dv, delta_ws, cu_q, cu_k, nseg, max_q, max_k, total_q, Hq, Hkv, D, strides16, scale, causal, dkv_ws,
+                                total_k, cos, sin, stream);
+}
diff --git a/rga3-release_amd/csrc/trainops.hip b/rga3-release_amd/csrc/trainops.hip
--- a/rga3-release_amd/csrc/trainops.hip
+++ b/rga3-release_amd/csrc/trainops.hip
@@ -49,10 +49,19 @@
     }
 }
 
-template <int NC>
-__global__ __launch_bounds__(256) void rmsnorm_bwd_block_kernel(const unsigned short* __restrict__ x, const unsigned short* __restrict__ w,
-                                                                const unsigned short* __restrict__ dy, const unsigned short* __restrict__ add,
-                                                                unsigned short* __restrict__ dx, int dim, float eps) {
+__device__ __forceinline__ unsigned dropout_hash(unsigned long long seed, unsigned long long ctr);
+
+struct Drop2 {
+    const unsigned short *ga, *gb;
+    unsigned thr_a, thr_b;
+    float ik_a, ik_b;
+    unsigned long long seed_a, seed_b;
+};
+
+template <int NC, bool DROP>
+__device__ __forceinline__ void rmsnorm_bwd_block_body(const unsigned short* __restrict__ x, const unsigned short* __restrict__ w,
+                                                       const unsigned short* __restrict__ dy, const unsigned short* __restrict__ add,
+                                                       unsigned short* __restrict__ dx, int dim, float eps, const Drop2& dr) {
     __shared__ float red[2][4];
     const int lane = threadIdx.x & 63, wv = threadIdx.x >> 6;
     const long row = blockIdx.x;
@@ -65,7 +74,21 @@
         if (ch < nch) {
             float fw[8];
             unpack8(*(const u32x4*)(x + row * dim + ch * 8), fx[i]);
-            unpack8(*(const u32x4*)(dy + row * dim + ch * 8), fg[i]);
+            u32x4 o = *(const u32x4*)(dy + row * dim + ch * 8);
+            if constexpr (DROP) {
+                const long g = row * nch + ch;
+                const u32x4 va = *(const u32x4*)(dr.ga + g * 8), vb = *(const u32x4*)(dr.gb + g * 8);
+#pragma unroll
+                for (int j = 0; j < 4; ++j) {
+                    const unsigned ha = dropout_hash(dr.seed_a, (unsigned long long)g * 4 + j), hb = dropout_hash(dr.seed_b, (unsigned long long)g * 4 + j);
+                    const float alo = ((ha & 0xffffu) >= dr.thr_a) ? __uint_as_float(va[j] << 16) * dr.ik_a : 0.f;
+                    const float ahi = ((ha >> 16) >= dr.thr_a) ? __uint_as_float(va[j] & 0xffff0000u) * dr.ik_a : 0.f;
+                    const float blo = ((hb & 0xffffu) >= dr.thr_b) ? __uint_as_float(vb[j] << 16) * dr.ik_b : 0.f;
+                    const float bhi = ((hb >> 16) >= dr.thr_b) ? __uint_as_float(vb[j] & 0xffff0000u) * dr.ik_b : 0.f;
+                    o[j] = pack_bf2(__uint_as_float(o[j] << 16) + alo + blo, __uint_as_float(o[j] & 0xffff0000u) + ahi + bhi);
+                }
+            }
+            unpack8(o, fg[i]);
             unpack8(*(const u32x4*)(w + ch * 8), fw);
 #pragma unroll
             for (int e = 0; e < 8; ++e) {
@@ -94,6 +117,18 @@
             *(u32x4*)(dx + row * dim + ch * 8) = pack8(o);
         }
     }
+}
+template <int NC>
+__global__ __launch_bounds__(256) void rmsnorm_bwd_block_kernel(const unsigned short* __restrict__ x, const unsigned short* __restrict__ w,
+                                                                const unsigned short* __restrict__ dy, const unsigned short* __restrict__ add,
+                                                                unsigned short* __restrict__ dx, int dim, float eps) {
+    rmsnorm_bwd_block_body<NC, false>(x, w, dy, add, dx, dim, eps, Drop2{});
+}
+template <int NC>
+__global__ __launch_bounds__(256) void rmsnorm_bwd_block_drop2_kernel(const unsigned short* __restrict__ x, const unsigned short* __restrict__ w,
+                                                                      const unsigned short* __restrict__ dy, const unsigned short* __restrict__ add,
+                                                                      unsigned short* __restrict__ dx, int dim, float eps, Drop2 dr) {
+    rmsnorm_bwd_block_body<NC, true>(x, w, dy, add, dx, dim, eps, dr);
 }
 
 __global__ __launch_bounds__(256) void swiglu_bwd_kernel(const unsigned short* __restrict__ gu, const unsigned short* __restrict__ da,
@@ -382,6 +417,23 @@
     return 0;
 }
 
+extern "C" int rga3_rmsnorm_bwd_drop2(const void* x, const void* weight, const void* dy, const void* add, void* dx, int64_t rows, int64_t dim, float eps,
+                                      const void* ga, const void* gb, float pa, int64_t seed_a, float pb, int64_t seed_b, void* stream) {
+    RGA3_CHECK_ARG(x && weight && dy && dx && ga && gb && rows > 0 && dim > 1024 && dim % 8 == 0 && dim <= 8192, "rmsnorm_bwd_drop2: bad args (1024 < dim <= 8192, dim %% 8)");
+    RGA3_CHECK_ARG(pa >= 0.f && pa < 1.f && pb >= 0.f && pb < 1.f, "rmsnorm_bwd_drop2: p=%f / %f", pa, pb);
+    RGA3_CHECK_ARG((((uintptr_t)x | (uintptr_t)weight | (uintptr_t)dy | (uintptr_t)add | (uintptr_t)dx | (uintptr_t)ga | (uintptr_t)gb) & 15) == 0,
+                   "rmsnorm_bwd_drop2: pointers must be 16-byte aligned");
+    const unsigned ta = (unsigned)(pa * 65536.0f + 0.5f), tb = (unsigned)(pb * 65536.0f + 0.5f);
+    const Drop2 dr{(cus)ga, (cus)gb, ta, tb, 1.0f / (1.0f - (float)ta / 65536.0f), 1.0f / (1.0f - (float)tb / 65536.0f), (unsigned long long)seed_a, (unsigned long long)seed_b};
+    hipStream_t st = (hipStream_t)stream;
+    dim3 gb_((unsigned)rows);
+    if (dim <= 2048) hipLaunchKernelGGL(rmsnorm_bwd_block_drop2_kernel<1>, gb_, dim3(256), 0, st, (cus)x, (cus)weight, (cus)dy, (cus)add, (us)dx, (int)dim, eps, dr);
+    else if (dim <= 4096) hipLaunchKernelGGL(rmsnorm_bwd_block_drop2_kernel<2>, gb_, dim3(256), 0, st, (cus)x, (cus)weight, (cus)dy, (cus)add, (us)dx, (int)dim, eps, dr);
+    else hipLaunchKernelGGL(rmsnorm_bwd_block_drop2_kernel<4>, gb_, dim3(256), 0, st, (cus)x, (cus)weight, (cus)dy, (cus)add, (us)dx, (int)dim, eps, dr);
+    RGA3_CHECK_LAUNCH("rmsnorm_bwd_block<drop2>");
+    return 0;
+}
+
 extern "C" int rga3_dropout_bf16(const void* x, void* y, int64_t n, float p, int64_t seed, int accumulate, void* stream) {
     RGA3_CHECK_ARG(x && y && n > 0 && n % 8 == 0, "dropout: n=%ld must be a positive multiple of 8", (long)n);
     RGA3_CHECK_ARG(p >= 0.f && p < 1.f, "dropout: p=%f", p);
diff --git a/rga3-release_amd/rga3/hip/lib.py b/rga3-release_amd/rga3/hip/lib.py
--- a/rga3-release_amd/rga3/hip/lib.py
+++ b/rga3-release_amd/rga3/hip/lib.py
@@ -58,6 +58,7 @@
     "rga3_stom_shift_composite": [_p, _p, _p, _p, _i64, _i64, _i64, _i, _p],
     "rga3_stom_mask_composite": [_p, _p, _p, _p, _p, _p, _i64, _i64, _i64, _i64, _i64, _i, _p, _i, _p, _i, _p],
     "rga3_attn_varlen_bwd": [_p, _p, _p, _p, _p, _p, _p, _p, _p, _p, _p, _p, _i, _i, _i, _i64, _i, _i, _i, _p, _f, _i, _p, _i64, _p],
+    "rga3_attn_varlen_bwd_rope": [_p, _p, _p, _p, _p, _p, _p, _p, _p, _p, _p, _p, _i, _i, _i, _i64, _i, _i, _i, _p, _f, _i, _p, _i64, _p, _p, _p],
     "rga3_transpose16_many": [_p, _p, _i, _p],
     "rga3_hiera_mlp144": [_p, _p, _p, _p, _p, _p, _p, _i64, _f, _p],
     "rga3_hiera_mlp288_pack_bytes": [],
@@ -85,6 +86,7 @@
     "rga3_qwen_norm_lut": [_p, _p, _i, _p],
     "rga3_qwen_patchify_u8": [_p, _i64, _i, _i, _p, _p, _i, _i, _i, _i, _p],
     "rga3_rmsnorm_bwd": [_p, _p, _p, _p, _p, _i64, _i64, _f, _p],
+    "rga3_rmsnorm_bwd_drop2": [_p, _p, _p, _p, _p, _i64, _i64, _f, _p, _p, _f, _i64, _f, _i64, _p],
     "rga3_dropout_bf16": [_p, _p, _i64, _f, _i64, _i, _p],
     "rga3_dropout_pair_bf16": [_p, _p, _p, _p, _i64, _f, _i64, _f, _i64, _i, _p],
     "rga3_swiglu_fwd": [_p, _p, _i64, _i64, _p],
diff --git a/rga3-release_amd/rga3/hip/ops.py b/rga3-release_amd/rga3/hip/ops.py
--- a/rga3-release_amd/rga3/hip/ops.py
+++ b/rga3-release_amd/rga3/hip/ops.py
@@ -961,7 +961,11 @@
     return out
 
 
-def attn_varlen_bwd(q, k, v, o, dout, lse, cu_q, cu_k, max_q: int, max_k: int, scale: float, causal: bool, dq=None, dk=None, dv=None):
+def attn_varlen_bwd_rope_ok(Hq: int, Hkv: int, D: int) -> bool:
+    return D % 32 == 0 and Hq > Hkv
+
+
+def attn_varlen_bwd(q, k, v, o, dout, lse, cu_q, cu_k, max_q: int, max_k: int, scale: float, causal: bool, dq=None, dk=None, dv=None, rope=None):
     import ctypes
     _need_cuda(q, k, v, o, dout, lse)
     Tq, Hq, D = q.shape
@@ -976,16 +980,39 @@
     dkv_ws = torch.empty((2 * Hq * Tk * D,), dtype=torch.float32, device=q.device) if (Hq > Hkv and D % 4 == 0) else None
     st = (ctypes.c_int64 * 16)(q.stride(0), q.stride(1), k.stride(0), k.stride(1), v.stride(0), v.stride(1), o.stride(0), o.stride(1),
                                dout.stride(0), dout.stride(1), dq.stride(0), dq.stride(1), dk.stride(0), dk.stride(1), dv.stride(0), dv.stride(1))
-    rc = _lib.load().rga3_attn_varlen_bwd(q.data_ptr(), k.data_ptr(), v.data_ptr(), o.data_ptr(), dout.data_ptr(), lse.data_ptr(), dq.data_ptr(),
-                                          dk.data_ptr(), dv.data_ptr(), delta.data_ptr(), cu_q.data_ptr(), cu_k.data_ptr(), cu_q.numel() - 1, int(max_q),
-                                          int(max_k), Tq, Hq, Hkv, D, ctypes.cast(st, ctypes.c_void_p), float(scale), int(bool(causal)), _ptr(dkv_ws), Tk, _stream())
-    _lib.check(rc, "attn_varlen_bwd")
+    args = (q.data_ptr(), k.data_ptr(), v.data_ptr(), o.data_ptr(), dout.data_ptr(), lse.data_ptr(), dq.data_ptr(), dk.data_ptr(), dv.data_ptr(), delta.data_ptr(),
+            cu_q.data_ptr(), cu_k.data_ptr(), cu_q.numel() - 1, int(max_q), int(max_k), Tq, Hq, Hkv, D, ctypes.cast(st, ctypes.c_void_p), float(scale), int(bool(causal)),
+            _ptr(dkv_ws), Tk)
+    if rope is not None:
+        cos, sin = rope
+        _need_cuda(cos, sin)
+        assert Tq == Tk and cos.dtype == sin.dtype == torch.float32 and cos.shape == sin.shape == (Tq, D) and cos.is_contiguous() and sin.is_contiguous()
+        if attn_varlen_bwd_rope_ok(Hq, Hkv, D):
+            _lib.check(_lib.load().rga3_attn_varlen_bwd_rope(*args, cos.data_ptr(), sin.data_ptr(), _stream()), "attn_varlen_bwd_rope")
+            return dq, dk, dv
+    _lib.check(_lib.load().rga3_attn_varlen_bwd(*args, _stream()), "attn_varlen_bwd")
+    if rope is not None:
+        if dk.data_ptr() == dq.data_ptr() + 2 * Hq * dq.stride(1) and dk.stride() == dq.stride():
+            rope_(dq.as_strided((Tq, Hq + Hkv, D), dq.stride()), cos, sin, 0, Hq + Hkv)
+        else:
+            rope_(dq, cos, sin, 0, Hq)
+            rope_(dk, cos, sin, 0, Hkv)
     return dq, dk, dv
 
 
-def rmsnorm_bwd(x, weight, dy, eps: float, add=None):
+def rmsnorm_bwd(x, weight, dy, eps: float, add=None, drop2=None):
     _need_cuda(x, weight, dy, add)
     assert x.is_contiguous() and dy.is_contiguous() and x.dtype == dy.dtype == torch.bfloat16 and (add is None or add.is_contiguous())
+    if drop2 is not None:
+        ga, pa, seed_a, gb, pb, seed_b = drop2
+        if x.shape[1] <= 1024:
+            return rmsnorm_bwd(x, weight, dropout_pair(ga, pa, seed_a, gb, pb, seed_b, accumulate_into=dy.clone()), eps, add=add)
+        _need_cuda(ga, gb)
+        assert ga.dtype == gb.dtype == torch.bfloat16 and ga.is_contiguous() and gb.is_contiguous() and ga.shape == gb.shape == dy.shape == x.shape
+        dx = torch.empty_like(x)
+        _lib.check(_lib.load().rga3_rmsnorm_bwd_drop2(x.data_ptr(), weight.data_ptr(), dy.data_ptr(), _ptr(add), dx.data_ptr(), x.shape[0], x.shape[1], float(eps),
+                                                      ga.data_ptr(), gb.data_ptr(), float(pa), int(seed_a), float(pb), int(seed_b), _stream()), "rmsnorm_bwd_drop2")
+        return dx
     dx = torch.empty_like(x)
     _lib.check(_lib.load().rga3_rmsnorm_bwd(x.data_ptr(), weight.data_ptr(), dy.data_ptr(), _ptr(add), dx.data_ptr(), x.shape[0], x.shape[1], float(eps),
                                             _stream()), "rmsnorm_bwd")
diff --git a/rga3-release_amd/rga3/model/qwen_train.py b/rga3-release_amd/rga3/model/qwen_train.py
--- a/rga3-release_amd/rga3/model/qwen_train.py
+++ b/rga3-release_amd/rga3/model/qwen_train.py
@@ -435,8 +435,7 @@
             datt = _fgemm(dx1, at, "wo_t", (at.o_proj.weight,), lambda: ops.transpose(at.o_proj.weight.detach())).view(T, Hq, D)
             dqkv = torch.empty_like(qkv)
             ops.attn_varlen_bwd(q, k, v, att, datt, lse, cu, cu, max_len, max_len, D ** -0.5, True, dq=dqkv[:, :Hq], dk=dqkv[:, Hq:Hq + Hk],
-                                dv=dqkv[:, Hq + Hk:])
-            ops.rope_(dqkv, cos, _neg_table(sin), 0, Hq + Hk)
+                                dv=dqkv[:, Hq + Hk:], rope=(cos, _neg_table(sin)))
             dqkv2 = dqkv.view(T, (Hq + 2 * Hk) * D)
             fold = (not _fp8["on"]) and T > 16 and _lora_cat_ok(at)
             dtt = None
@@ -446,6 +445,7 @@
             else:
                 dh1 = _fgemm(dqkv2, at, "wqkv_t", (at.q_proj.weight, at.k_proj.weight, at.v_proj.weight), lambda: ops.transpose(wqkv))
             grads = [None, None, None, None]
+            drop2 = None
             if lq is not None or lv is not None:
                 tn_pairs, tn_slots = [], []
                 pend = []
@@ -467,13 +467,13 @@
                     else:
                         pend.append((ops.gemm(dt, At), pdrop, ctx.seeds[sd]))
                 if len(pend) == 2 and dh1.is_contiguous():
-                    ops.dropout_pair(pend[0][0], pend[0][1], pend[0][2], pend[1][0], pend[1][1], pend[1][2], accumulate_into=dh1)
+                    drop2 = (pend[0][0], pend[0][1], pend[0][2], pend[1][0], pend[1][1], pend[1][2])
                 else:
                     for xg, pg, sg in pend:
                         ops.dropout(xg, pg, sg, out=dh1, accumulate=True)
                 for sl, gw in zip(tn_slots, ops.gemm_tn_many(tn_pairs)):
                     grads[sl] = gw
-            dx = ops.rmsnorm_bwd(x, w1.weight, dh1, w1.variance_epsilon, add=dx1)
+            dx = ops.rmsnorm_bwd(x, w1.weight, dh1, w1.variance_epsilon, add=dx1, drop2=drop2)
         return (dx, grads[0], grads[1], grads[2], grads[3], None, None, None, None, None, None)
 
 
```

Result: no change. 7.486 (-0.9%).
